# deryrahman/image-caption-emotion-indonesia

Hardware: AMD Instinct MI355X
Metric: images/sec (train step) + NLL loss match, batch=64 ResNet152+FactoredLSTM-512 (higher is better)
Workload: dtype f32 (trunk: operands as 2 f16 pieces each, 3 MFMA products per multiply, f32 accumulate; decoder: large products as 3 bf16 pieces per operand, 6 MFMA products per multiply, the rest f32 MFMA; the persistent LSTM kernel the trunk's split-f16 scheme)

## Files before the change

image-caption-emotion-indonesia_amd/_lib.py:

```python
import ctypes as C
import os

_HERE = os.path.dirname(os.path.abspath(__file__))
LIB_PATH = os.path.join(_HERE, "libcapnet_hip.so")

_f = C.POINTER(C.c_float)
_vp = C.c_void_p
_i = C.c_int
_l = C.c_long
_sz = C.c_size_t
_ip = C.POINTER(C.c_int)

SIGNATURES = {
    "capnet_last_error": (C.c_char_p, []),
    "capnet_abi_version": (_i, []),
    "capnet_sgemm": (_i, [_i, _i, _i, _i, _i, _vp, _l, _vp, _l, _vp, _l, _vp, _i, _i, _l, _l, _l,
                          _l, _i, _vp]),
    "capnet_sgemm_b3": (_i, [_i, _i, _i, _i, _i, _vp, _l, _vp, _l, _vp, _l, _vp, _i, _i, _l, _l, _l, _l, _vp, _sz, _vp]),
    "capnet_sgemm_b3_eligible": (_i, [_i, _i, _i, _i, _i, _vp, _l, _vp, _l, _vp, _l, _vp, _i, _l, _l, _l, _l]),
    "capnet_sgemm_splitk": (_i, [_i, _i, _i, _i, _i, _vp, _l, _vp, _l, _vp, _l, _vp, _i, _vp, _sz, _vp]),
    "capnet_sgemm_splitk_fused": (_i, [_i, _i, _i, _i, _i, _vp, _l, _vp, _l, _vp, _l, _vp, _i, _vp, _sz, _vp, _sz, _vp]),
    "capnet_colsum": (_i, [_vp, _l, _i, _i, _vp, _i, _vp]),
    "capnet_argmax_rows": (_i, [_vp, _i, _i, _i, _vp, _vp]),
    "capnet_resize_u8": (_i, [_vp, _i, _i, _vp, _vp, _i, _i, _vp, _vp, _i, _vp, _vp, _i, _vp]),
    "capnet_crop_flip_normalize": (_i, [_vp, _i, _i, _i, _vp, _vp, _i, _i, _f, _f, _vp]),
    "capnet_topk_correct": (_i, [_vp, _l, _i, _i, _vp, _i, _vp, _vp, _vp]),
    "capnet_beam_topk": (_i, [_vp, _l, _i, _i, _vp, _i, _vp, _vp, _vp]),
    "capnet_beam_topk_batched": (_i, [_vp, _l, _i, _vp, _vp, _i, _vp, _vp, _vp]),
    "capnet_beam_state_bytes": (_sz, [_i, _i, _i]),
    "capnet_beam_init": (_i, [_vp, _i, _i, _i, C.c_longlong, _vp, _vp]),
    "capnet_beam_advance": (_i, [_vp, _vp, _l, _i, _i, _i, _i, _i, C.c_longlong, _vp, _vp, _vp]),
    "capnet_beam_finish": (_i, [_vp, _i, _i, _i, C.c_longlong, _vp, _vp, _vp]),
    "capnet_beam_live": (_i, [_vp, _i, _i, _i, C.POINTER(_vp), C.POINTER(_vp), C.POINTER(_vp)]),
    "capnet_att_step_fwd": (_i, [_vp, _vp, _vp, _vp, _l, _vp, _vp, _i, _i, _i, _i, _vp, _vp, _i, _i,
                                 _vp, _vp, _l, _vp, _vp]),
    "capnet_trunk_create": (_i, [_i, _i, _i, C.POINTER(_vp)]),
    "capnet_trunk_destroy": (None, [_vp]),
    "capnet_trunk_workspace_bytes": (_sz, [_vp]),
    "capnet_trunk_num_convs": (_i, [_vp]),
    "capnet_trunk_final_side": (_i, [_vp]),
    "capnet_trunk_flops": (C.c_double, [_vp]),
    "capnet_trunk_conv_flops": (C.c_double, [_vp, _i]),
    "capnet_trunk_conv_shape": (_i, [_vp, _i, _ip, _ip, _ip, _ip, _ip]),
    "capnet_trunk_forward": (_i, [_vp, _vp, C.POINTER(_vp), C.POINTER(_vp), C.POINTER(_vp),
                                  C.POINTER(_vp), C.POINTER(_vp), _i, C.c_float, C.c_float, _vp,
                                  _vp, _vp, _ip, _vp, _vp]),
    "capnet_trunk_set_tail_balance": (_i, [_vp, _i]),
    "capnet_trunk_update_running": (_i, [_vp, _vp, C.POINTER(_vp), C.POINTER(_vp), C.c_float, _vp]),
    "capnet_pack_conv_weight": (_i, [_vp, _vp, _i, _i, _i, _i, _i, _vp]),
    "capnet_adaptive_pool_replicate": (_i, [_vp, _vp, _i, _i, _i, _i, _vp]),
    "capnet_conv2d_fwd": (_i, [_vp, _l, _l, _l, _l, _vp, _i, _vp, _vp, _vp, _i, _vp, _vp, _i, _i,
                               _i, _i, _i, _i, _i, _i, _i, _i, _vp]),
    "capnet_trunk_conv_kmajor": (_i, [_vp, _i]),
    "capnet_trunk_conv_tile_n": (_i, [_vp, _i]),
    "capnet_pack_conv_weight_kmajor": (_i, [_vp, _vp, _i, _i, _i, _i, _i, _vp]),
    "capnet_conv2d_fwd_kmajor": (_i, [_vp, _l, _l, _l, _vp, _i, _vp, _vp, _vp, _i, _vp, _vp, _i, _i,
                                      _i, _i, _i, _i, _i, _i, _i, _i, _vp, _vp]),
    "capnet_sgemm_nt_dma_eligible": (_i, [_i, _i, _i, _vp, _l, _vp, _l, _vp, _l]),
    "capnet_sgemm_nt_dma": (_i, [_i, _i, _i, _vp, _l, _vp, _vp, _vp, _vp]),
    "capnet_conv1x1_tiles_m": (_i, [_l]),
    "capnet_conv1x1_fwd_dma": (_i, [_vp, _l, _l, _l, _vp, _vp, _vp, _vp, _i, _i, _i, _i, _i, _i, _vp, _vp,
                                    _vp, _i, _vp]),
    "capnet_conv1x1_f16x3_weight_words": (_sz, [_i, _i]),
    "capnet_conv1x1_f16x3_bn": (_i, [_l, _i]),
    "capnet_conv1x1_f16x3_pack": (_i, [_vp, _vp, _i, _i, _i, _vp]),
    "capnet_conv1x1_fwd_f16x3": (_i, [_vp, _l, _l, _l, _vp, _i, _vp, _vp, _vp, _i, _vp, _vp, _i, _i, _i, _i, _i,
                                      _i, _vp, _vp, _vp, _i, _vp]),
    "capnet_conv3x3_fwd_patch": (_i, [_vp, _vp, _i, _vp, _vp, _vp, _i, _vp, _vp, _i, _i, _i, _i, _i, _i, _vp]),
    "capnet_conv1x1_fwd_tail": (_i, [_vp, _vp, _vp, _vp, _vp, _vp, _vp, _vp, _i, _vp, _vp, _vp, _l, _i, _i, _vp]),
    "capnet_conv2d_fwd_f16x3_scaled": (_i, [_vp, _l, _l, _l, _vp, _i, _vp, _vp, _vp, _i, _vp, _vp, _i, _i, _i, _i, _i,
                                            _i, _i, _i, _i, _vp]),
    "capnet_conv3x3_fwd_patch_scaled": (_i, [_vp, _vp, _i, _vp, _vp, _vp, _i, _vp, _vp, _i, _i, _i, _i, _i, _i, _i, _vp]),
    "capnet_conv1x1_fwd_tail_scaled": (_i, [_vp, _vp, _vp, _vp, _vp, _vp, _vp, _vp, _i, _vp, _vp, _vp, _l, _i, _i, _i, _vp]),
    "capnet_conv_stem_f16x3_weight_words": (_sz, []),
    "capnet_conv_stem_f16x3_part_rows": (_i, [_i, _i, _i]),
    "capnet_conv_stem_f16x3_pack": (_i, [_vp, _vp, _vp]),
    "capnet_conv_stem_fwd_f16x3": (_i, [_vp, _l, _l, _l, _vp, _vp, _vp, _vp, _i, _i, _i, _vp]),
    "capnet_conv_f16x3_weight_words": (_sz, [_i, _i, _i]),
    "capnet_conv_f16x3_pack": (_i, [_vp, _vp, _i, _i, _i, _i, _vp]),
    "capnet_conv2d_fwd_f16x3": (_i, [_vp, _l, _l, _l, _vp, _i, _vp, _vp, _vp, _i, _vp, _vp, _i, _i, _i, _i, _i,
                                     _i, _i, _i, _vp, _vp, _vp, _i, _vp]),
    "capnet_conv_kmajor_slab_floats": (_sz, [_i, _i, _i, _i]),
    "capnet_conv_kmajor_plan": (None, [_i, _i, _i, _i, _ip]),
    "capnet_conv_kmajor_tiles_m": (_i, [_i, _i, _i, _i]),
    "capnet_conv_tiles_m": (_i, [_i, _i, _i]),
    "capnet_bn_finalize": (_i, [_vp, _vp, _i, _i, _l, _vp, _vp, _vp, _vp, C.c_float, C.c_float,
                                _vp, _vp, _vp]),
    "capnet_bn_add_relu": (_i, [_vp, _vp, _vp, _vp, _vp, _vp, _vp, _l, _i, _vp]),
    "capnet_bn_relu_maxpool": (_i, [_vp, _vp, _vp, _vp, _i, _i, _i, _i, _vp]),
    "capnet_global_avgpool": (_i, [_vp, _vp, _i, _i, _i, _vp]),
    "capnet_bn1d_fwd": (_i, [_vp, _i, _i, _vp, _vp, _vp, _vp, _i, C.c_float, C.c_float, _vp, _vp,
                             _vp, _vp]),
    "capnet_bn1d_bwd": (_i, [_vp, _vp, _i, _i, _vp, _vp, _vp, _vp, _vp, _vp, _vp]),
    "capnet_seq_saved_floats": (_sz, [_ip]),
    "capnet_seq_saved_ints": (_sz, [_ip]),
    "capnet_seq_saved_cell_offset": (_sz, [_ip]),
    "capnet_seq_fwd_scratch_floats": (_sz, [_ip]),
    "capnet_seq_bwd_scratch_floats": (_sz, [_ip]),
    "capnet_seq_forward": (_i, [_ip, _ip, C.POINTER(C.c_ubyte), _vp, _vp, _vp, C.POINTER(_vp),
                                _vp, _vp, C.c_float, C.c_ulonglong, _i, _vp, _vp, _vp, _vp, _vp,
                                _vp]),
    "capnet_seq_backward": (_i, [_ip, _ip, _vp, _vp, _vp, _vp, _vp, C.POINTER(_vp), C.c_float,
                                 C.c_ulonglong, _i, _vp]),
    "capnet_seq_forward_stacked": (_i, [_ip, _i, _ip, _vp, _vp, _vp, _vp, C.POINTER(_vp), _vp, _vp, C.c_float, C.c_ulonglong, _i,
                                        C.POINTER(_vp), C.POINTER(_vp), _vp, C.POINTER(_vp), _vp, _vp]),
    "capnet_seq_backward_stacked": (_i, [_ip, _i, _ip, _vp, C.POINTER(_vp), C.POINTER(_vp), C.POINTER(_vp), _vp, C.POINTER(_vp),
                                         C.POINTER(_vp), C.c_float, C.c_ulonglong, _i, _vp]),
    "capnet_att_saved_floats": (_sz, [_ip]),
    "capnet_att_saved_ints": (_sz, [_ip]),
    "capnet_att_fwd_scratch_floats": (_sz, [_ip]),
    "capnet_att_bwd_scratch_floats": (_sz, [_ip]),
    "capnet_att_seq_forward": (_i, [_ip, _ip, C.POINTER(C.c_ubyte), _vp, _vp, _vp, C.POINTER(_vp),
                                    _vp, _vp, C.c_float, C.c_ulonglong, _i, _vp, _vp, _vp, _vp, _vp,
                                    _vp, _vp]),
    "capnet_att_seq_backward": (_i, [_ip, _ip, _vp, _vp, _vp, _vp, C.POINTER(_vp), _vp, _vp, _vp,
                                     C.POINTER(_vp), C.c_float, C.c_ulonglong, _i, _vp]),
    "capnet_att_stacked_saved_floats": (_sz, [_ip, _i]),
    "capnet_att_stacked_saved_ints": (_sz, [_ip, _i]),
    "capnet_att_stacked_fwd_scratch_floats": (_sz, [_ip, _i]),
    "capnet_att_stacked_bwd_scratch_floats": (_sz, [_ip, _i]),
    "capnet_att_seq_forward_stacked": (_i, [_ip, _i, _ip, C.POINTER(C.c_ubyte), _vp, _vp, _vp, C.POINTER(_vp), _vp, _vp,
                                            C.c_float, C.c_ulonglong, _i, C.POINTER(_vp), C.POINTER(_vp), _vp,
                                            C.POINTER(_vp), _vp, _vp, _vp]),
    "capnet_att_seq_backward_stacked": (_i, [_ip, _i, _ip, _vp, _vp, C.POINTER(_vp), _vp, C.POINTER(_vp), C.POINTER(_vp),
                                             C.POINTER(_vp), _vp, C.POINTER(_vp), C.POINTER(_vp), C.c_float,
                                             C.c_ulonglong, _i, _vp]),
    "capnet_embedding_fwd": (_i, [_vp, _i, _vp, _i, _i, _vp, _vp, _vp]),
    "capnet_lstm_pointwise_fwd": (_i, [_vp, _vp, _vp, _vp, _i, _i, _i, _vp]),
    "capnet_stacked_decode_step": (_i, [_i, _i, _i, _i, _i, _vp, _vp, C.POINTER(_vp), C.POINTER(_vp), _vp, _vp, _vp, _vp,
                                        _vp]),
    "capnet_stacked_decode_step_cell": (_i, [_i, _i, _i, _i, _i, _i, _vp, _vp, C.POINTER(_vp), C.POINTER(_vp), _vp, _vp,
                                             _vp, _vp, _vp]),
    "capnet_stacked_decode_step_gather": (_i, [_i, _i, _i, _i, _i, _i, _vp, _vp, C.POINTER(_vp), C.POINTER(_vp), _vp, _vp,
                                               _vp, _vp, _vp, _vp]),
    "capnet_stacked_decode_step_groups": (_i, [_i, _i, _i, _i, _i, _i, _i, _vp, _vp, C.POINTER(_vp), C.POINTER(_vp), _vp, _vp,
                                               _vp, _vp, _vp, _vp]),
    "capnet_stacked_decode_step_tables": (_i, [_i, _i, _i, _i, _i, _i, _i, _vp, C.POINTER(_vp), C.POINTER(_vp), C.POINTER(_vp),
                                               _vp, _vp, _vp, _vp, _vp, _vp]),
    "capnet_vocab_argmax_ws_bytes": (_sz, [_i, _i]),
    "capnet_vocab_argmax_groups_ws_bytes": (_sz, [_i, _i, _i]),
    "capnet_vocab_argmax_groups": (_i, [_vp, C.POINTER(_vp), C.POINTER(_vp), _i, _i, _i, _i, _vp, _vp, _vp]),
    "capnet_vocab_argmax": (_i, [_vp, _vp, _vp, _i, _i, _i, _vp, _vp, _vp]),
    "capnet_lstm_greedy_decode_ws_bytes": (_sz, [_i, _i, _i, _i]),
    "capnet_lstm_greedy_decode": (_i, [_i, _i, _i, _i, _i, _i, _vp, _vp, _vp, C.POINTER(_vp), C.POINTER(_vp), _vp, _vp, _vp,
                                       _vp, _vp, _vp, _vp, _vp]),
    "capnet_lstm_greedy_decode_groups_ws_bytes": (_sz, [_i, _i, _i, _i, _i]),
    "capnet_lstm_greedy_decode_groups": (_i, [_i, _i, _i, _i, _i, _i, _i, _vp, C.POINTER(_vp), C.POINTER(_vp), C.POINTER(_vp),
                                              C.POINTER(_vp), C.POINTER(_vp), _vp, _vp, _vp, _vp, _vp, _vp]),
    "capnet_beam_decode_ws_bytes": (_sz, [_i, _i, _i, _i, _i, _i]),
    "capnet_beam_decode": (_i, [_i, _i, _i, _i, _i, _i, _i, _i, C.c_longlong, C.c_longlong, _vp, C.POINTER(_vp),
                                C.POINTER(_vp), _vp, _vp, _vp, _vp, _vp, _sz, _i, _vp, _vp, C.POINTER(_i), _vp, _vp]),
    "capnet_beam_decode_groups": (_i, [_i, _i, _i, _i, _i, _i, _i, _i, _i, C.c_longlong, C.c_longlong, _vp, C.POINTER(_vp),
                                       C.POINTER(_vp), _vp, _vp, _vp, _vp, _vp, _sz, _i, _vp, _vp, C.POINTER(_i), _vp, _vp]),
    "capnet_vocab_topk_ws_bytes": (_sz, [_i, _i, _i]),
    "capnet_vocab_topk": (_i, [_vp, _vp, _vp, _i, _i, _i, _i, _vp, _vp, _vp, _vp, _vp]),
    "capnet_sample_uniform": (C.c_float, [C.c_ulonglong, C.c_uint, C.c_uint, C.c_uint]),
    "capnet_vocab_sample_ws_bytes": (_sz, [_i, _i]),
    "capnet_vocab_sample": (_i, [_vp, _vp, _vp, _i, _i, _i, C.c_float, C.c_ulonglong, C.c_uint, C.c_uint, _vp, _vp, _vp, _vp]),
    "capnet_vocab_sample_greedy": (_i, [_vp, _vp, _vp, _i, _i, _i, C.c_float, C.c_ulonglong, C.c_uint, C.c_uint, _vp, _vp, _vp, C.c_uint, _vp]),
    "capnet_sample_pick": (_i, [_vp, _vp, _i, _i, _i, C.c_float, C.c_ulonglong, C.c_uint, C.c_uint, _vp, _vp, _vp]),
    "capnet_sample_pick_greedy": (_i, [_vp, _vp, _i, _i, _i, C.c_float, C.c_ulonglong, C.c_uint, C.c_uint, _vp, _vp, C.c_uint, _vp]),
    "capnet_sample_rows": (_i, [_vp, _i, _l, _i, C.c_float, C.c_ulonglong, C.c_uint, C.c_uint, _vp, _vp, _vp]),
    "capnet_sample_rows_greedy": (_i, [_vp, _i, _l, _i, C.c_float, C.c_ulonglong, C.c_uint, C.c_uint, _vp, _vp, C.c_uint, _vp]),
    "capnet_sample_decode_ws_bytes": (_sz, [_i, _i, _i, _i, _i]),
    "capnet_sample_decode": (_i, [_i, _i, _i, _i, _i, _i, _i, _vp, _vp, _vp, C.POINTER(_vp), C.POINTER(_vp), _vp, _vp, _vp,
                                  C.c_float, _i, C.c_ulonglong, _vp, _vp, _vp, _vp, _vp, _vp]),
    "capnet_sample_decode_greedy": (_i, [_i, _i, _i, _i, _i, _i, _i, _vp, _vp, _vp, C.POINTER(_vp), C.POINTER(_vp), _vp, _vp, _vp,
                                  C.c_float, _i, C.c_ulonglong, _vp, _vp, _vp, _vp, _vp, C.c_uint, _vp]),
    "capnet_att_sample_decode_ws_bytes": (_sz, [_i] * 10),
    "capnet_att_sample_decode": (_i, [_i] * 11 + [_vp] * 8 + [C.POINTER(_vp), C.POINTER(_vp), _vp, _vp, _vp, C.c_float, _i,
                                                            C.c_ulonglong, _vp, _vp, _sz, _vp, _vp, _vp, _vp, _vp]),
    "capnet_att_sample_decode_greedy": (_i, [_i] * 11 + [_vp] * 8 + [C.POINTER(_vp), C.POINTER(_vp), _vp, _vp, _vp, C.c_float, _i,
                                                            C.c_ulonglong, _vp, _vp, _sz, _vp, _vp, _vp, _vp, C.c_uint, _vp]),
    "capnet_nucleus_rows": (_i, [_vp, _i, _l, _i, C.c_float, C.c_float, C.c_ulonglong, C.c_uint, C.c_uint, _vp, _vp, _vp]),
    "capnet_nucleus_rows_greedy": (_i, [_vp, _i, _l, _i, C.c_float, C.c_float, C.c_ulonglong, C.c_uint, C.c_uint, _vp, _vp, C.c_uint, _vp]),
    "capnet_nucleus_pick": (_i, [_vp, _vp, _i, _i, _i, C.c_float, C.c_float, C.c_ulonglong, C.c_uint, C.c_uint, _vp, _vp, _vp]),
    "capnet_nucleus_pick_greedy": (_i, [_vp, _vp, _i, _i, _i, C.c_float, C.c_float, C.c_ulonglong, C.c_uint, C.c_uint, _vp, _vp, C.c_uint, _vp]),
    "capnet_sample_decode_nucleus_ws_bytes": (_sz, [_i, _i, _i, _i, _i]),
    "capnet_sample_decode_nucleus": (_i, [_i, _i, _i, _i, _i, _i, _i, _vp, _vp, _vp, C.POINTER(_vp), C.POINTER(_vp), _vp, _vp, _vp,
                                          C.c_float, _i, C.c_float, C.c_ulonglong, _vp, _vp, _sz, _vp, _vp, _vp, _vp, _vp]),
    "capnet_sample_decode_nucleus_greedy": (_i, [_i, _i, _i, _i, _i, _i, _i, _vp, _vp, _vp, C.POINTER(_vp), C.POINTER(_vp), _vp, _vp, _vp,
                                          C.c_float, _i, C.c_float, C.c_ulonglong, _vp, _vp, _sz, _vp, _vp, _vp, _vp, C.c_uint, _vp]),
    "capnet_att_sample_decode_nucleus_ws_bytes": (_sz, [_i] * 10),
    "capnet_att_sample_decode_nucleus": (_i, [_i] * 11 + [_vp] * 8 + [C.POINTER(_vp), C.POINTER(_vp), _vp, _vp, _vp, C.c_float, _i,
                                                                    C.c_float, C.c_ulonglong, _vp, _vp, _sz, _vp, _vp, _vp, _vp,
                                                                    _vp]),
    "capnet_att_sample_decode_nucleus_greedy": (_i, [_i] * 11 + [_vp] * 8 + [C.POINTER(_vp), C.POINTER(_vp), _vp, _vp, _vp, C.c_float, _i,
                                                                    C.c_float, C.c_ulonglong, _vp, _vp, _sz, _vp, _vp, _vp, _vp,
                                                                    C.c_uint, _vp]),
    "capnet_vocab_topk_groups_ws_bytes": (_sz, [_i, _i, _i, _i]),
    "capnet_vocab_topk_groups": (_i, [_vp, C.POINTER(_vp), C.POINTER(_vp), _i, _i, _i, _i, _i, _vp, _vp, _vp, _vp, _vp]),
    "capnet_beam_advance_topk": (_i, [_vp, _vp, _vp, _vp, _i, _i, _i, _i, _i, C.c_longlong, _vp, _vp, _vp]),
    "capnet_lstm_beam_decode_ws_bytes": (_sz, [_i, _i, _i, _i, _i, _i, _i]),
    "capnet_lstm_beam_decode": (_i, [_i, _i, _i, _i, _i, _i, _i, _i, C.c_longlong, C.c_longlong, _vp, _vp, C.POINTER(_vp),
                                     C.POINTER(_vp), _vp, _vp, _vp, _vp, _vp, _sz, _i, _i, _vp, _vp, C.POINTER(_i), _vp, _vp]),
    "capnet_lstm_beam_decode_groups_ws_bytes": (_sz, [_i, _i, _i, _i, _i, _i, _i, _i]),
    "capnet_lstm_beam_decode_groups": (_i, [_i, _i, _i, _i, _i, _i, _i, _i, _i, C.c_longlong, C.c_longlong, C.POINTER(_vp),
                                            C.POINTER(_vp), C.POINTER(_vp), C.POINTER(_vp), C.POINTER(_vp), _vp, _vp, _vp, _sz,
                                            _i, _i, _vp, _vp, C.POINTER(_i), _vp, _vp]),
    "capnet_att_decode_supported": (_i, [_i, _i, _i, _i, _i, _i, _i]),
    "capnet_att_decode_step_ws_bytes": (_sz, [_i, _i, _i, _i, _i, _i]),
    "capnet_att_decode_step": (_i, [_i] * 10 + [_vp] * 8 + [C.POINTER(_vp), C.POINTER(_vp), _vp, _vp, _vp, _vp, _vp, _vp, _sz,
                                                          _vp, _vp]),
    "capnet_att_decode_step_groups": (_i, [_i] * 11 + [_vp] * 8 + [C.POINTER(_vp), C.POINTER(_vp), _vp, _vp, _vp, _vp, _vp, _vp,
                                                                 _sz, _vp, _vp]),
    "capnet_att_beam_decode_ws_bytes": (_sz, [_i] * 10),
    "capnet_att_beam_decode": (_i, [_i] * 11 + [C.c_longlong, C.c_longlong] + [_vp] * 7 + [C.POINTER(_vp), C.POINTER(_vp), _vp,
                                                                                           _vp, _vp, _vp, _vp, _sz, _i, _vp, _vp,
                                                                                           C.POINTER(_i), _vp, _vp]),
    "capnet_att_beam_decode_groups": (_i, [_i] * 12 + [C.c_longlong, C.c_longlong] + [_vp] * 7 + [C.POINTER(_vp), C.POINTER(_vp),
                                                                                                  _vp, _vp, _vp, _vp, _vp, _sz,
                                                                                                  _i, _vp, _vp, C.POINTER(_i),
                                                                                                  _vp, _vp]),
    "capnet_beam_trace_bytes": (_sz, [_i, _i, _i]),
    "capnet_beam_advance_traced": (_i, [_vp, _vp, _vp, _l, _i, _i, _i, _i, _i, C.c_longlong, _vp, _vp, _vp]),
    "capnet_beam_finish_traced": (_i, [_vp, _vp, _i, _i, _i, C.c_longlong, _vp, _vp, _vp, _vp]),
    "capnet_att_decode_step_alphas": (_i, [_i] * 11 + [_vp] * 8 + [C.POINTER(_vp), C.POINTER(_vp), _vp, _vp, _vp, _vp, _vp, _vp,
                                                                 _sz, _vp, _vp, _vp]),
    "capnet_att_beam_decode_alphas_ws_bytes": (_sz, [_i] * 11),
    "capnet_att_beam_decode_alphas": (_i, [_i] * 12 + [C.c_longlong, C.c_longlong] + [_vp] * 7 + [C.POINTER(_vp), C.POINTER(_vp),
                                                                                                  _vp, _vp, _vp, _vp, _vp, _sz,
                                                                                                  _i, _vp, _vp, C.POINTER(_i),
                                                                                                  _vp, _vp, _vp]),
    "capnet_beam_nbest": (_i, [_vp, _i, _i, _i, C.c_float, _vp, _vp, _vp, _vp, _vp]),
    "capnet_beam_nbest_traced": (_i, [_vp, _vp, _i, _i, _i, C.c_float, _vp, _vp, _vp, _vp, _vp, _vp]),
    "capnet_beam_decode_ws_beam_offset": (_sz, [_i] * 8),
    "capnet_att_beam_decode_alphas_ws_trace_offset": (_sz, [_i] * 11),
    "capnet_att_beam_decode_alphas_ws_hist_offset": (_sz, [_i] * 11),
    "capnet_alpha_gather": (_i, [_vp, _vp, _i, _i, _i, _i, _vp, _vp]),
    "capnet_lstm_wfrag_floats": (_sz, [_i]),
    "capnet_lstm_pack_wfrag": (_i, [_vp, _vp, _i, _i, _vp]),
    "capnet_lstm_step_fused": (_i, [_vp, _vp, _vp, _l, _vp, _vp, _vp, _i, _i, _i, _vp]),
    "capnet_lstm_step_fused_stamped": (_i, [_vp, _vp, _vp, _l, _vp, _vp, _vp, _i, _i, _vp, _vp]),
    "capnet_lstm_step_fused_supported": (_i, [_i, _i]),
    "capnet_lstm_persist_supported": (_i, [_i, _i]),
    "capnet_lstm_persist_w_floats": (_sz, []),
    "capnet_lstm_persist_ctl_ints": (_sz, []),
    "capnet_lstm_persist_pack": (_i, [_vp, _vp, _i, _vp]),
    "capnet_lstm_persist_run": (_i, [_vp, _vp, _vp, _vp, _ip, _i, _i, _i, _i, _i, _vp, _vp, _vp, _vp]),
    "capnet_xent_fwd": (_i, [_vp, _l, _i, _i, _vp, _vp, _vp, _vp, _vp, _vp]),
    "capnet_xent_bwd": (_i, [_vp, _l, _i, _i, _vp, _vp, _vp, _vp, _l, _vp]),
    "capnet_att_loss_fwd": (_i, [_vp, _vp, _i, _i, _i, C.c_float, _vp, _vp, _vp]),
    "capnet_att_loss_bwd": (_i, [_vp, _vp, _i, _i, _i, C.c_float, _vp, _vp]),
    "capnet_policy_xent_fwd": (_i, [_vp, _l, _i, _i, _vp, _vp, _i, _ip, _i, _vp, _vp, _vp, _vp, _vp, _vp]),
    "capnet_policy_xent_bwd": (_i, [_vp, _l, _i, _i, _vp, _vp, _vp, _i, _ip, _i, _vp, _vp, _l, _vp]),
    "capnet_bleu_rows": (_i, [_vp, _l, _i, _i, C.c_longlong, C.c_longlong, _i, _vp, _vp, _i, _i, _i, C.POINTER(C.c_double), _i,
                              _vp, _vp, _vp]),
    "capnet_cider_rows": (_i, [_vp, _l, _i, _i, C.c_longlong, C.c_longlong, _i, _vp, _vp, _vp, _i, _i, _i, C.POINTER(_vp),
                               C.POINTER(_vp), _ip, C.c_double, C.c_double, _vp, _vp, _vp, _vp]),
    "capnet_clamp_adam": (_i, [_i, C.POINTER(_vp), C.POINTER(_vp), C.POINTER(_vp),
                               C.POINTER(_vp), C.POINTER(_l), _ip, C.c_float, C.c_float,
                               C.c_float, C.c_float, C.c_float, _i, _vp, _vp]),
    "capnet_lstm_persist_set_mode": (_i, [_i]),
    "capnet_att_set_chain_mode": (_i, [_i]),
    "capnet_lstm_pointwise_bwd": (_i, [_vp, _vp, _vp, _vp, _vp, _vp, _i, _i, _i, _vp]),
    "capnet_conv1x1_fwd_areg": (_i, [_vp, _vp, _i, _vp, _vp, _vp, _i, _vp, _vp, _l, _i, _i, _i, _vp]),
    "capnet_trunk_set_timing": (_i, [_vp, _i]),
    "capnet_trunk_time_next_pass": (_i, [_vp]),
    "capnet_trunk_collect_timing": (_i, [_vp, C.POINTER(C.c_double), C.POINTER(_l),
                                         C.POINTER(C.c_double)]),
    "capnet_packed_targets": (_i, [_vp, _i, _i, _ip, _vp, _vp]),
    "capnet_fused_block_weight_words": (_sz, [_i, _i, _i]),
    "capnet_fused_block_pack": (_i, [_vp, _vp, _i, _i, _i, _vp]),
    "capnet_fused_block_stats_floats": (_sz, [_l, _i]),
    "capnet_fused_block_stats": (_i, [_vp, _vp, _vp, _vp, _l, _i, _i, _vp, _vp, _vp, _vp, C.c_float, C.c_float, _vp, _vp, _vp,
                                      _vp, _vp]),
    "capnet_fused_block_tiles": (_i, [_l, _i]),
    "capnet_fused_block_forward": (_i, [_vp] * 14 + [_l, _i, _i, _i, _vp, _vp]),
    "capnet_comm_unique_id": (_i, [_vp]),
    "capnet_comm_create": (_i, [_vp, _i, _i, C.POINTER(_vp)]),
    "capnet_comm_destroy": (_i, [_vp]),
    "capnet_allreduce_grads": (_i, [_vp, _vp, _l, _vp]),
    "capnet_err_word_exchange": (_i, [_vp, _vp, _i, _vp]),
    "capnet_count_skipped": (_i, [_vp, _vp, _vp]),
    "capnet_pack_tensors": (_i, [_i, C.POINTER(_vp), C.POINTER(_l), _vp, _i, C.c_float, _vp]),
    "capnet_clamp": (_i, [_vp, _l, C.c_float, C.c_float, _vp]),
}


class CapnetError(RuntimeError):
    pass


_lib = None


def lib():
    global _lib
    if _lib is None:
        if not os.path.exists(LIB_PATH):
            raise CapnetError(
                "libcapnet_hip.so is not built (%s). Run `python -c 'import __graft_entry__ as g; "
                "g.build()'` or `make -C image-caption-emotion-indonesia_amd/csrc`. There is no "
                "CPU fallback." % LIB_PATH)
        l = C.CDLL(LIB_PATH)
        for name, (res, args) in SIGNATURES.items():
            fn = getattr(l, name)
            fn.restype = res
            fn.argtypes = args
        _lib = l
    return _lib


def check(status, what=""):
    if status != 0:
        msg = lib().capnet_last_error()
        raise CapnetError("%s failed (status %d): %s" %
                          (what or "capnet call", status, msg.decode() if msg else "?"))


def ptr(t):
    if t is None:
        return None
    return C.c_void_p(t.data_ptr())


def ptr_array(tensors):
    arr = (C.c_void_p * len(tensors))()
    for k, t in enumerate(tensors):
        arr[k] = None if t is None else t.data_ptr()
    return arr


def int_array(vals):
    return (C.c_int * len(vals))(*[int(v) for v in vals])


def current_stream():
    import torch
    return C.c_void_p(torch.cuda.current_stream().cuda_stream)
```

image-caption-emotion-indonesia_amd/csrc/capi.cpp:

```cpp
#include "../../include/capnet.h"

#include "common.h"
#include "kernels.h"

using namespace capnet;

static inline hipStream_t S(capnet_stream_t s) { return reinterpret_cast<hipStream_t>(s); }

static SeqDims to_dims(const int* d) {
  SeqDims r;
  r.B = d[0]; r.T = d[1]; r.steps = d[2]; r.N = d[3]; r.E = d[4]; r.F = d[5]; r.H = d[6];
  r.V = d[7]; r.has_features = d[8]; r.cell = d[9];
  return r;
}

static bool weight_used(int cell, int i) { return cell == kCellFactored || i == 0 || i == 4 || i == 24 || i == 28; }
template <class Weights>
static void to_weights(const float* const* weights, Weights& w) {
  for (int g = 0; g < 4; ++g) {
    w.Vw[g] = weights[0 + g];  w.Vb[g] = weights[4 + g];
    w.Sw[g] = weights[8 + g];  w.Sb[g] = weights[12 + g];
    w.Uw[g] = weights[16 + g]; w.Ub[g] = weights[20 + g];
    w.Ww[g] = weights[24 + g]; w.Wb[g] = weights[28 + g];
  }
// ... 1087 lines not shown
int capnet_att_sample_decode_nucleus_greedy(int cell, int nlayers, int n, int m, int P, int A, int C, int E, int H, int V,
                                            int steps, const long long* start_tokens, const float* att1, const float* feat,
                                            const float* emb, const float* wz, const float* bz, const float* w_full,
                                            const float* b_full, const float* const* wcat, const float* const* beff,
                                            const float* Cw, const float* Cb, const float* state0, float temperature,
                                            int top_k, float top_p, unsigned long long seed, void* workspace, float* slab,
                                            size_t slab_floats, long long* ids, float* logp, float* state_out, int* err_flag,
                                            unsigned greedy_stride, capnet_stream_t stream) {
  return att_sample_decode_nucleus_tail(cell, nlayers, n, m, P, A, C, E, H, V, steps, start_tokens, att1, feat, emb, wz, bz,
                                        w_full, b_full, wcat, beff, Cw, Cb, state0, temperature, top_k, top_p, seed,
                                        workspace, slab, slab_floats, ids, logp, state_out, err_flag, stream, greedy_stride);
}

size_t capnet_att_beam_decode_alphas_ws_bytes(int nlayers, int groups, int n, int k, int P, int A, int C, int E, int H, int V,
                                              int max_steps) {
  return att_beam_decode_alphas_ws_bytes(nlayers, groups, n, k, P, A, C, E, H, V, max_steps);
}

int capnet_att_beam_decode_alphas(int cell, int nlayers, int groups, int n, int k, int P, int A, int C, int E, int H, int V,
                                  int max_steps, long long start_token, long long end_token, const float* att1,
                                  const float* feat, const float* emb, const float* wz, const float* bz, const float* w_full,
                                  const float* b_full, const float* const* wcat, const float* const* beff, const float* Cw,
                                  const float* Cb, const float* state0, void* workspace, float* slab, size_t slab_floats,
                                  int poll_every, long long* seqs, int* lengths, int* steps_run, int* err_flag,
                                  capnet_stream_t stream, float* alphas) {
  return att_beam_decode_entry(cell, nlayers, groups, n, k, P, A, C, E, H, V, max_steps, start_token, end_token, att1, feat, emb, wz,
                               bz, w_full, b_full, wcat, beff, Cw, Cb, state0, workspace, slab, slab_floats, poll_every, seqs,
                               lengths, steps_run, err_flag, stream, true, alphas);
}

int capnet_lstm_pointwise_bwd(const float* gates, const float* c, const float* c_prev, const float* dh, float* dc_io,
                              float* dpre, int b, int H, int cell, capnet_stream_t stream) {
  CAPNET_REQUIRE(gates && c && dh && dc_io && dpre && b >= 0 && H > 0, "lstm_pointwise_bwd: bad argument");
  CAPNET_REQUIRE(cell == kCellFactored || cell == kCellLSTM, "lstm_pointwise_bwd: unknown cell %d", cell);
  const bool f = cell == kCellFactored;
  return lstm_pointwise_bwd(gates, 4L * H, c, c_prev, dh, nullptr, dc_io, dpre, 4L * H, b, b, H, 0, 1, f ? 2 : 3, f ? 3 : 2,
                            f ? 0 : 1, S(stream), 0, 0);
}
size_t capnet_lstm_wfrag_floats(int H) { return lstm_wfrag_floats(H); }
int capnet_lstm_pack_wfrag(const float* w_cat, float* w_frag, int H, int cell, capnet_stream_t stream) {
  CAPNET_REQUIRE(cell == kCellFactored || cell == kCellLSTM, "lstm_pack_wfrag: unknown cell %d", cell);
  return cell == kCellFactored ? lstm_pack_wfrag(w_cat, w_frag, H, 0, 1, 2, 3, S(stream))
                               : lstm_pack_wfrag(w_cat, w_frag, H, 0, 1, 3, 2, S(stream));
}
int capnet_lstm_step_fused(const float* h_prev, const float* w_cat, float* gates, long ldg,
                           const float* c_prev, float* c_out, float* h_out, int b, int H, int cell,
                           capnet_stream_t stream) {
  CAPNET_REQUIRE(cell == kCellFactored || cell == kCellLSTM, "lstm_step_fused: unknown cell %d", cell);
  if (cell == kCellFactored)
    return lstm_step_fused(h_prev, w_cat, gates, ldg, c_prev, c_out, h_out, b, H, 0, 1, 2, 3, 0, S(stream));
  return lstm_step_fused(h_prev, w_cat, gates, ldg, c_prev, c_out, h_out, b, H, 0, 1, 3, 2, 1, S(stream));
}
int capnet_lstm_step_fused_stamped(const float* h_prev, const float* w_frag, float* gates, long ldg,
                                   const float* c_prev, float* c_out, float* h_out, int b, int H,
                                   unsigned long long* stamps, capnet_stream_t stream) {
  return lstm_step_fused(h_prev, w_frag, gates, ldg, c_prev, c_out, h_out, b, H, 0, 1, 2, 3, 0,
                         S(stream), stamps);
}
int capnet_lstm_step_fused_supported(int b, int H) { return lstm_step_fused_supported(b, H) ? 1 : 0; }

int capnet_lstm_persist_supported(int b, int H) { return lstm_persist_supported(b, H) ? 1 : 0; }
int capnet_lstm_persist_set_mode(int mode) { return lstm_persist_set_mode(mode); }
size_t capnet_lstm_persist_w_floats(void) { return lstm_persist_w_floats(); }
size_t capnet_lstm_persist_ctl_ints(void) { return lstm_persist_ctl_ints(); }
int capnet_lstm_persist_pack(const float* w_cat, float* w_img, int cell, capnet_stream_t stream) {
  CAPNET_REQUIRE(cell == kCellFactored || cell == kCellLSTM, "lstm_persist_pack: unknown cell %d", cell);
  return cell == kCellFactored ? lstm_persist_pack(w_cat, w_img, 0, 1, 2, 3, S(stream))
                               : lstm_persist_pack(w_cat, w_img, 0, 1, 3, 2, S(stream));
}
int capnet_lstm_persist_run(const float* w_img, float* gates, float* cell_states, float* hiddens,
                            const int* batch_sizes, int t0, int t1, int H, int cell, int segment,
                            int* ctl, int* err_flag, unsigned long long* stamps,
                            capnet_stream_t stream) {
  CAPNET_REQUIRE(cell == kCellFactored || cell == kCellLSTM, "lstm_persist_run: unknown cell %d", cell);
  CAPNET_REQUIRE(batch_sizes && t1 > 0 && t1 <= kMaxSteps, "lstm_persist_run: bad steps");
  int off[kMaxSteps + 1];
  off[0] = 0;
  for (int t = 0; t < t1; ++t) off[t + 1] = off[t] + batch_sizes[t];
  const bool f = cell == kCellFactored;
  return lstm_persist_run(w_img, gates, cell_states, hiddens, off, batch_sizes, t0, t1, H, 0, 1,
                          f ? 2 : 3, f ? 3 : 2, f ? 0 : 1, segment, ctl, err_flag, S(stream), stamps);
}

size_t capnet_seq_saved_floats(const int* dims) { return seq_saved_floats(to_dims(dims)); }
size_t capnet_seq_saved_ints(const int* dims) { return seq_saved_ints(to_dims(dims)); }
size_t capnet_seq_saved_cell_offset(const int* dims) { return seq_saved_cell_offset(to_dims(dims)); }
size_t capnet_seq_fwd_scratch_floats(const int* dims) { return seq_fwd_scratch_floats(to_dims(dims)); }
size_t capnet_seq_bwd_scratch_floats(const int* dims) { return seq_bwd_scratch_floats(to_dims(dims)); }

int capnet_seq_forward_stacked(const int* dims, int nlayers, const int* batch_sizes, const unsigned char* tf_mask,
                               const long long* captions, const float* features, const float* emb,
                               const float* const* weights, const float* Cw, const float* Cb, float dropout_p,
                               unsigned long long seed, int training, float* const* saved, int* const* saved_i,
                               float* scratch, float* const* hiddens, int* err_flag, capnet_stream_t stream) {
  CAPNET_REQUIRE(dims && weights && nlayers >= 1 && nlayers <= 8, "seq_forward_stacked: null dims / weights or layers %d", nlayers);
  const SeqDims d = to_dims(dims);
  CAPNET_REQUIRE(d.cell == kCellFactored || d.cell == kCellLSTM, "seq_forward_stacked: unknown cell %d", d.cell);
  SeqWeights w[8];
  for (int l = 0; l < nlayers; ++l) {
    for (int i = 0; i < 32; ++i)
      CAPNET_REQUIRE(!weight_used(d.cell, i) || weights[32 * l + i], "seq_forward_stacked: weight %d of layer %d is null", i, l);
    to_weights(weights + 32 * l, w[l]);
  }
  return seq_forward_stacked(d, nlayers, batch_sizes, tf_mask, captions, features, emb, w, Cw, Cb, dropout_p, seed, training,
                             saved, saved_i, scratch, hiddens, err_flag, S(stream));
}

int capnet_seq_backward_stacked(const int* dims, int nlayers, const int* batch_sizes, const float* d_hiddens,
                                const float* const* hiddens, const float* const* saved, const int* const* saved_i,
                                float* scratch, float* const* dh_work, float* const* grads, float dropout_p,
                                unsigned long long seed, int training, capnet_stream_t stream) {
  CAPNET_REQUIRE(dims && grads && nlayers >= 1 && nlayers <= 8, "seq_backward_stacked: null dims / grads or layers %d", nlayers);
  SeqGrads g[8];
  for (int l = 0; l < nlayers; ++l) to_grads(grads + 9 * l, g[l]);
  return seq_backward_stacked(to_dims(dims), nlayers, batch_sizes, d_hiddens, hiddens, saved, saved_i, scratch, dh_work, g,
                              dropout_p, seed, training, S(stream));
}

int capnet_seq_forward(const int* dims, const int* batch_sizes, const unsigned char* tf_mask,
                       const long long* captions, const float* features, const float* emb,
                       const float* const* weights, const float* Cw, const float* Cb,
                       float dropout_p, unsigned long long seed, int training, float* saved,
                       int* saved_i, float* scratch, float* hiddens, int* err_flag,
                       capnet_stream_t stream) {
  return capnet_seq_forward_stacked(dims, 1, batch_sizes, tf_mask, captions, features, emb, weights, Cw, Cb, dropout_p, seed,
                                    training, &saved, &saved_i, scratch, &hiddens, err_flag, stream);
}

int capnet_seq_backward(const int* dims, const int* batch_sizes, const float* d_hiddens,
                        const float* hiddens, const float* saved, const int* saved_i,
                        float* scratch, float* const* grads, float dropout_p,
                        unsigned long long seed, int training, capnet_stream_t stream) {
  return capnet_seq_backward_stacked(dims, 1, batch_sizes, d_hiddens, &hiddens, &saved, &saved_i, scratch, nullptr, grads,
                                     dropout_p, seed, training, stream);
}

int capnet_att_set_chain_mode(int mode) { return att_set_chain_mode(mode); }
size_t capnet_att_saved_floats(const int* dims) { return att_saved_floats(to_adims(dims)); }
size_t capnet_att_saved_ints(const int* dims) { return att_saved_ints(to_adims(dims)); }
size_t capnet_att_fwd_scratch_floats(const int* dims) { return att_fwd_scratch_floats(to_adims(dims)); }
size_t capnet_att_bwd_scratch_floats(const int* dims) { return att_bwd_scratch_floats(to_adims(dims)); }

int capnet_beam_topk_batched(const float* logits, long ld, int V, const float* prev_scores, const int* meta, int n,
                             float* top_scores, long long* top_index, capnet_stream_t stream) {
  return beam_topk_batched(logits, ld, V, prev_scores, meta, n, top_scores, top_index, S(stream));
}
int capnet_beam_topk(const float* logits, long ld, int rows, int V, const float* prev_scores, int k,
                     float* top_scores, long long* top_index, capnet_stream_t stream) {
  return beam_topk(logits, ld, rows, V, prev_scores, k, top_scores, top_index, S(stream));
}
size_t capnet_beam_state_bytes(int n, int k, int max_steps) { return beam_state_bytes(n, k, max_steps); }
int capnet_beam_init(void* beam, int n, int k, int max_steps, long long start_token, long long* prev_words,
                     capnet_stream_t stream) {
  return beam_init(beam, n, k, max_steps, start_token, prev_words, S(stream));
}
int capnet_beam_advance(void* beam, const float* logits, long ld, int V, int n, int k, int max_steps, int step,
                        long long end_token, long long* next_words, long long* parent_rows, capnet_stream_t stream) {
  return beam_advance(beam, logits, ld, V, n, k, max_steps, step, end_token, next_words, parent_rows, S(stream));
}
int capnet_beam_advance_topk(void* beam, const float* values, const int* index, const float* lse, int V, int n, int k,
                             int max_steps, int step, long long end_token, long long* next_words, long long* parent_rows,
                             capnet_stream_t stream) {
  return beam_advance_topk(beam, values, index, lse, V, n, k, max_steps, step, end_token, next_words, parent_rows, S(stream));
}
int capnet_beam_finish(const void* beam, int n, int k, int max_steps, long long end_token, long long* seqs, int* lengths,
                       capnet_stream_t stream) {
  return beam_finish(beam, n, k, max_steps, end_token, seqs, lengths, S(stream));
}
size_t capnet_beam_trace_bytes(int n, int k, int max_steps) { return beam_trace_bytes(n, k, max_steps); }
int capnet_beam_advance_traced(void* beam, void* trace, const float* logits, long ld, int V, int n, int k, int max_steps,
                               int step, long long end_token, long long* next_words, long long* parent_rows,
                               capnet_stream_t stream) {
  CAPNET_REQUIRE(trace != nullptr, "beam_advance_traced: null trace");
  CAPNET_REQUIRE((size_t)beam % 4 == 0 && (size_t)trace % 4 == 0, "beam_advance_traced: the state and the trace must be 4-byte aligned");
  return beam_advance(beam, logits, ld, V, n, k, max_steps, step, end_token, next_words, parent_rows, S(stream), trace);
}
int capnet_beam_finish_traced(const void* beam, const void* trace, int n, int k, int max_steps, long long end_token,
                              long long* seqs, int* lengths, int* rows, capnet_stream_t stream) {
  CAPNET_REQUIRE(trace && rows, "beam_finish_traced: null trace or rows");
  CAPNET_REQUIRE((size_t)beam % 4 == 0 && (size_t)trace % 4 == 0 && (size_t)rows % 4 == 0,
                 "beam_finish_traced: the state, the trace and the rows must be 4-byte aligned");
  return beam_finish(beam, n, k, max_steps, end_token, seqs, lengths, S(stream), trace, rows);
}
int capnet_beam_nbest(const void* beam, int n, int k, int max_steps, float length_penalty, long long* seqs, int* lengths,
                      float* scores, int* counts, capnet_stream_t stream) {
  return beam_nbest(beam, n, k, max_steps, length_penalty, seqs, lengths, scores, counts, S(stream));
}
int capnet_beam_nbest_traced(const void* beam, const void* trace, int n, int k, int max_steps, float length_penalty,
                             long long* seqs, int* lengths, float* scores, int* counts, int* rows, capnet_stream_t stream) {
  CAPNET_REQUIRE(trace && rows, "beam_nbest_traced: null trace or rows");
  CAPNET_REQUIRE((size_t)beam % 4 == 0 && (size_t)trace % 4 == 0 && (size_t)rows % 4 == 0,
                 "beam_nbest_traced: the state, the trace and the rows must be 4-byte aligned");
  return beam_nbest(beam, n, k, max_steps, length_penalty, seqs, lengths, scores, counts, S(stream), trace, rows);
}
size_t capnet_beam_decode_ws_beam_offset(int nlayers, int n, int k, int H, int V, int max_steps, int fused_topk, int groups) {
  return beam_decode_ws_beam_offset(nlayers, n, k, H, V, max_steps, fused_topk, groups);
}
size_t capnet_att_beam_decode_alphas_ws_trace_offset(int nlayers, int groups, int n, int k, int P, int A, int C, int E, int H,
                                                     int V, int max_steps) {
// ... 250 lines not shown
```

image-caption-emotion-indonesia_amd/csrc/decoder_seq.cpp:

```cpp
#include <vector>

#include "common.h"
#include "kernels.h"

#include "seq_layers.h"

namespace capnet {

namespace seqd {

std::vector<int> step_offsets(const int* batch_sizes, int steps) {
  std::vector<int> off(steps + 1, 0);
  for (int t = 0; t < steps; ++t) off[t + 1] = off[t] + batch_sizes[t];
  return off;
}

std::vector<int> with_state_step(int B, const int* batch_sizes, int steps) {
  std::vector<int> bse(steps + 1, B);
  for (int t = 0; t < steps; ++t) bse[t + 1] = batch_sizes[t];
  return bse;
}

int check_batch_sizes(const char* who, const int* batch_sizes, int steps, int B, int N) {
  CAPNET_REQUIRE(batch_sizes != nullptr, "%s: null batch_sizes", who);
  long n = 0;
  int prev = B;
  for (int t = 0; t < steps; ++t) {
    CAPNET_REQUIRE(batch_sizes[t] > 0 && batch_sizes[t] <= prev,
                   "%s: batch_sizes must be positive and non-increasing (step %d: %d after %d)", who, t, batch_sizes[t], prev);
    prev = batch_sizes[t];
    n += batch_sizes[t];
  }
  CAPNET_REQUIRE(n == N, "%s: sum(batch_sizes)=%ld != N=%d", who, n, N);
  return kOk;
}

int build_row_tables(const std::vector<int>& off, const unsigned char* tf_mask, int has_features, bool lead, int* row_sample,
                     int* row_col, int* row_token, int* prev_row, hipStream_t s) {
  SeqMeta m;
  m.steps = (int)off.size() - 1; m.N = off.back(); m.has_features = has_features;
  for (int t = 0; t <= m.steps; ++t) m.off[t] = off[t];
  if (lead) m.tf[0] = 1;
  for (int t = lead; t < m.steps; ++t) m.tf[t] = tf_mask[t - lead] ? 1 : 0;
  return build_rows(m, row_sample, row_col, row_token, prev_row, s);
}

Layout make_layout(const SeqDims& d) {
  Layout L;
  Carve take, itake;
  const size_t N = d.N, E = d.E, F = d.F, H = d.H;
  L.X = take(N * E);
  L.G = take(N * 4 * H);
  L.Cst = take(N * H);
  L.Wcat = take(4 * H * H);
  L.Wfrag = take(H % 16 == 0 ? lstm_wfrag_floats((int)H) : 4);
  L.Wp = take(H == 512 ? lstm_persist_w_floats() : 4);
  L.bUW = take(4 * H);
  if (d.cell == kCellFactored) {
    L.A1 = take(N * 4 * F);
    L.A2 = take(N * 4 * F);
    L.Vcat = take(4 * F * E);
    L.Scat = take(4 * F * F);
    L.Ucat = take(4 * H * F);
    L.bV = take(4 * F);
    L.bS = take(4 * F);
  } else {
    L.A1 = L.A2 = L.Scat = L.Ucat = L.bV = L.bS = 0;
    L.Vcat = take(4 * H * E);
  }
  L.total = take.o;
  L.row_sample = itake(N);
  L.row_col = itake(N);
  L.row_token = itake(N);
  L.prev_row = itake(N);
  L.ctl = itake(lstm_persist_ctl_ints());
  L.itotal = itake.o;
  return L;
}

BwdLayout make_bwd_layout(const SeqDims& d, int lead) {
  BwdLayout S;
  Carve take;
  const size_t N = d.N, F = d.F, H = d.H;
  const bool fac = d.cell == kCellFactored;
  S.dPre = take(N * 4 * H);
  S.Hprev = take(N * H);
  S.dh_rec = take((size_t)d.B * H);
  S.dc = take((size_t)d.B * H);
  S.dX = take(N * d.E);
  S.dA2 = take(fac ? N * 4 * F : 0);
  S.dA1 = take(fac ? N * 4 * F : 0);
  S.skws = take(kSplitKFloats);
  S.A1c = take(fac && lead ? N * 4 * F : 0);
  S.A2c = take(fac && lead ? N * 4 * F : 0);
  S.total = take.o;
  return S;
}

int check_dims(const SeqDims& d, const int* batch_sizes) {
  CAPNET_REQUIRE(d.B > 0 && d.T > 0 && d.steps > 0 && d.N > 0 && d.E > 0 && d.H > 0 && d.V > 0,
                 "decoder: bad dims B=%d T=%d steps=%d N=%d E=%d H=%d V=%d", d.B, d.T, d.steps, d.N, d.E, d.H, d.V);
  CAPNET_REQUIRE(d.cell == kCellLSTM || d.F > 0, "decoder: factored size");
  RC(check_batch_sizes("decoder", batch_sizes, d.steps, d.B, d.N));
  CAPNET_REQUIRE(d.steps <= d.T + (d.has_features ? 1 : 0),
                 "decoder: %d steps need more caption columns than T=%d", d.steps, d.T);
  return kOk;
}

int copy_d2d(float* dst, const float* src, size_t n, hipStream_t s) {
  CAPNET_HIP_CHECK(hipMemcpyAsync(dst, src, n * sizeof(float), hipMemcpyDeviceToDevice, s));
  return kOk;
}

static size_t nctr(const SkWs& k) { return k.ctr ? kSplitKCounters : 0; }

int chain_fwd(const Chain& c, const float* X, int n, float* A1, float* A2, float* out, long ldo, const float* bias, int accumulate,
              const SkWs& k, hipStream_t s) {
  const int XW = c.XW, F = c.F, H = c.H;
  RC(sgemm_splitk(false, true, n, 4 * F, XW, X, XW, c.Vcat, XW, A1, 4 * F, c.bV, 0, k.ws, k.floats, s, k.ctr, nctr(k)));
  RC(sgemm_splitk_batched(false, true, n, F, F, A1, 4 * F, c.Scat, F, A2, 4 * F, c.bS, 0, 4, F, (long)F * F, F, F, k.ws, k.floats,
                          s, k.ctr, nctr(k)));
  return sgemm_splitk_batched(false, true, n, H, F, A2, 4 * F, c.Ucat, F, out, ldo, bias, accumulate, 4, F, (long)H * F, H,
                              bias ? H : 0, k.ws, k.floats, s, k.ctr, nctr(k));
}

int chain_collapse(const Chain& c, float* US, float* Weff, float* c1, float* bias, const SkWs& k, hipStream_t s) {
  const int XW = c.XW, F = c.F, H = c.H;
  RC(sgemm(false, false, H, F, F, c.Ucat, F, c.Scat, F, US, F, nullptr, 0, 4, (long)H * F, (long)F * F, (long)H * F, 0, 0, s));
  RC(sgemm(false, false, H, XW, F, US, F, c.Vcat, XW, Weff, XW, nullptr, 0, 4, (long)H * F, (long)F * XW, (long)H * XW, 0, 0, s));
  RC(sgemm_splitk_batched(false, true, 1, F, F, c.bV, F, c.Scat, F, c1, F, c.bS, 0, 4, F, (long)F * F, F, F, k.ws, k.floats, s,
                          k.ctr, nctr(k)));
  return sgemm_splitk_batched(false, true, 1, H, F, c1, F, c.Ucat, F, bias, H, nullptr, 1, 4, F, (long)H * F, H, 0, k.ws, k.floats,
                              s, k.ctr, nctr(k));
}

int chain_rows(const Chain& c, const float* X, int n, float* A1, float* A2, const SkWs& k, hipStream_t s) {
  const int XW = c.XW, F = c.F;
  RC(sgemm_splitk(false, true, n, 4 * F, XW, X, XW, c.Vcat, XW, A1, 4 * F, c.bV, 0, k.ws, k.floats, s, k.ctr, nctr(k)));
  return sgemm(false, true, n, F, F, A1, 4 * F, c.Scat, F, A2, 4 * F, c.bS, 0, 4, F, (long)F * F, F, F, 0, s);
}

int chain_bwd_rows(const Chain& c, const float* dG, long ldg, int n, float* dA2, float* dA1, hipStream_t s) {
  const int F = c.F, H = c.H;
  RC(sgemm(false, false, n, F, H, dG, ldg, c.Ucat, F, dA2, 4 * F, nullptr, 0, 4, H, (long)H * F, F, 0, 0, s));
  return sgemm(false, false, n, F, F, dA2, 4 * F, c.Scat, F, dA1, 4 * F, nullptr, 0, 4, F, (long)F * F, F, 0, 0, s);
}

int chain_wgrads(const Chain& c, const float* dG, long ldg, const float* X, const float* A1, const float* A2, const float* dA2,
                 const float* dA1, int n, const ChainGrads& g, hipStream_t s) {
  const int XW = c.XW, F = c.F, H = c.H;
  RC(sgemm(true, false, H, F, n, dG, ldg, A2, 4 * F, g.dUcat, F, nullptr, 0, 4, H, F, (long)H * F, 0, 0, s));
  RC(colsum(dA2, 4 * F, n, 4 * F, g.dbS, 0, s));
  RC(sgemm(true, false, F, F, n, dA2, 4 * F, A1, 4 * F, g.dScat, F, nullptr, 0, 4, F, F, (long)F * F, 0, 0, s));
  RC(colsum(dA1, 4 * F, n, 4 * F, g.dbV, 0, s));
  return sgemm(true, false, 4 * F, XW, n, dA1, 4 * F, X, XW, g.dVcat, XW, nullptr, 0, 1, 0, 0, 0, 0, 0, s);
}

int lstm_input_wgrad(const float* dG, long ldg, const float* X, int XW, int H, int n, float* dWih, hipStream_t s) {
  return sgemm(true, false, 4 * H, XW, n, dG, ldg, X, XW, dWih, XW, nullptr, 0, 1, 0, 0, 0, 0, 0, s);
}

int input_chain(const SeqDims& d, const Layout& L, float* sv, int r0, int r1, const SkWs& k, hipStream_t s) {
  const int n = r1 - r0;
  if (n <= 0) return kOk;
  const int E = d.E, F = d.F, H = d.H;
  const SkWs kn{n <= 128 ? k.ws : nullptr, k.floats, k.ctr};
  const float* X = sv + L.X + (size_t)r0 * E;
  float* G = sv + L.G + (size_t)r0 * 4 * H;
  if (d.cell == kCellFactored)
    return chain_fwd(chain_of(d, L, sv), X, n, sv + L.A1 + (size_t)r0 * 4 * F, sv + L.A2 + (size_t)r0 * 4 * F, G, 4 * H, sv + L.bUW,
                     0, kn, s);
  return sgemm_splitk(false, true, n, 4 * H, E, X, E, sv + L.Vcat, E, G, 4 * H, sv + L.bUW, 0, kn.ws, kn.floats, s, kn.ctr, nctr(kn));
}

int init_state(const float* mean, int B, int H, int C, const UpperInit& w, float* h0, float* c0, const SkWs& k, hipStream_t s) {
  RC(sgemm_splitk(false, true, B, H, C, mean, C, w.init_h_w, C, h0, H, w.init_h_b, 0, k.ws, k.floats, s, k.ctr, nctr(k)));
  return sgemm_splitk(false, true, B, H, C, mean, C, w.init_c_w, C, c0, H, w.init_c_b, 0, k.ws, k.floats, s, k.ctr, nctr(k));
// ... 78 lines not shown
  return kOk;
}

static bool between_layers(int training, float dropout_p) {
  return (training & 1) && !(training & kSeqInputDropoutOnly) && dropout_p > 0.f;
}

SeqDims upper_dims(const SeqDims& d0) {
  SeqDims d = d0;
  d.E = d0.H;
  d.has_features = 0;
  return d;
}
}

SeqDims seq_upper_dims(const SeqDims& d0) { return upper_dims(d0); }

int seq_forward_stacked(const SeqDims& d0, int nlayers, const int* batch_sizes, const unsigned char* tf_mask,
                        const long long* captions, const float* features, const float* emb, const SeqWeights* w,
                        const float* Cw, const float* Cb, float dropout_p, unsigned long long seed, int training,
                        float* const* saved, int* const* saved_i, float* scratch, float* const* hiddens, int* err_flag,
                        hipStream_t s) {
  RC(check_dims(d0, batch_sizes));
  CAPNET_REQUIRE(nlayers >= 1 && nlayers <= 8 && w && saved && saved_i && hiddens, "seq_forward_stacked: bad argument");
  CAPNET_REQUIRE(tf_mask && captions && emb && scratch && err_flag, "seq_forward: null argument");
  CAPNET_REQUIRE(!d0.has_features || features, "seq_forward: features missing");
  CAPNET_REQUIRE(dropout_p >= 0.f && dropout_p < 1.f, "seq_forward: dropout p=%f", dropout_p);
  const int E = d0.E, N = d0.N, H = d0.H;
  bool any_free = false;
  for (int t = 1; t < d0.steps; ++t) any_free |= !tf_mask[t];
  CAPNET_REQUIRE(!any_free || (Cw && Cb), "seq_forward: output projection needed for free-running steps");
  CAPNET_REQUIRE(d0.steps <= kMaxSteps, "seq_forward: %d steps > %d", d0.steps, kMaxSteps);
  const std::vector<int> off = step_offsets(batch_sizes, d0.steps);

  std::vector<LayerCtx> lay(nlayers);
  for (int l = 0; l < nlayers; ++l) {
    CAPNET_REQUIRE(saved[l] && saved_i[l] && hiddens[l], "seq_forward: null buffer of layer %d", l);
    lay[l].d = l == 0 ? d0 : upper_dims(d0);
    lay[l].L = make_layout(lay[l].d);
    lay[l].sv = saved[l]; lay[l].svi = saved_i[l]; lay[l].hid = hiddens[l];
    RC(build_row_tables(off, tf_mask, d0.has_features, false, lay[l].svi + lay[l].L.row_sample, lay[l].svi + lay[l].L.row_col,
                        lay[l].svi + lay[l].L.row_token, lay[l].svi + lay[l].L.prev_row, s));
    RC(pack_layer(lay[l], w[l], batch_sizes, s));
  }
  LayerCtx& c0 = lay[0];
  LayerCtx& top = lay[nlayers - 1];

  CAPNET_HIP_CHECK(hipMemsetAsync(c0.sv + c0.L.X, 0, (size_t)N * E * sizeof(float), s));
  RC(gather_inputs(captions, d0.T, features, emb, E, d0.V, c0.svi + c0.L.row_sample, c0.svi + c0.L.row_col,
                   c0.svi + c0.L.row_token, c0.sv + c0.L.X, E, 0, N, dropout_p, seed, training && dropout_p > 0.f, 0,
                   err_flag, s));
  float* skws = scratch + (size_t)d0.B * d0.V + 64;
  int* skctr = reinterpret_cast<int*>(skws + kSplitKWs);
  const SkWs sk{skws, kSplitKWs, skctr};
  CAPNET_HIP_CHECK(hipMemsetAsync(skctr, 0, kSplitKCounters * sizeof(int), s));
  RC(input_chain(c0.d, c0.L, c0.sv, 0, N, sk, s));
  const Feedback fb{captions, features, emb, Cw, Cb, d0.T, E, d0.V, H, dropout_p, seed, c0.svi + c0.L.row_sample,
                    c0.svi + c0.L.row_col, c0.svi + c0.L.row_token, scratch, err_flag};

  for (int t = 0; t < d0.steps;) {
    int t1 = t + 1;
    while (t1 < d0.steps && tf_mask[t1]) ++t1;
    const int b = batch_sizes[t], r0 = off[t], r1 = off[t1];
    if (t > 0 && !tf_mask[t]) {
      RC(feed_back(fb, top.hid + (size_t)off[t - 1] * H, b, r0, c0.sv + c0.L.X, E, sk, s));
      RC(input_chain(c0.d, c0.L, c0.sv, r0, r0 + b, sk, s));
    }
    for (int l = 0; l < nlayers; ++l) {
      LayerCtx& c = lay[l];
      if (l > 0) {
        RC(rows_dropout(lay[l - 1].hid, c.sv + c.L.X, r0, r1, H, dropout_p, seed, l, between_layers(training, dropout_p), s));
        RC(input_chain(c.d, c.L, c.sv, r0, r1, sk, s));
      }
      RC(recur(c, off, batch_sizes, t, t1, skws, skctr, err_flag, s));
    }
    t = t1;
  }
  return kOk;
}

static int seq_backward_layer(const SeqDims& d, const int* batch_sizes, const float* dH, const float* hiddens,
                              const float* saved, const int* saved_i, float* scratch, const SeqGrads& g,
                              float dropout_p, unsigned long long seed, int training, int layer, float* dH_below,
                              hipStream_t s, int lead = 0, float* dh0 = nullptr, float* dc0 = nullptr) {
  RC(check_dims(d, batch_sizes));
  CAPNET_REQUIRE(dH && hiddens && saved && saved_i && scratch, "seq_backward: null argument");
  CAPNET_REQUIRE(g.dWcat && g.dbUW && g.dVcat && (layer > 0 ? dH_below != nullptr : g.dEmb != nullptr), "seq_backward: null gradient buffer");
  CAPNET_REQUIRE(lead == 0 || (layer > 0 && d.steps > 1 && dh0 && dc0), "seq_backward: leading state step");
  const Layout L = make_layout(d);
  const BwdLayout S = make_bwd_layout(d, lead);
  const int E = d.E, F = d.F, H = d.H, N = d.N;
  const bool fac = d.cell == kCellFactored;
  const GateOrder go = gate_order(d.cell);
  const std::vector<int> off = step_offsets(batch_sizes, d.steps);
  const int R0 = off[lead], Nr = N - R0;
  float *dPre = scratch + S.dPre, *Hprev = scratch + S.Hprev, *dh_rec = scratch + S.dh_rec, *dc = scratch + S.dc;
  float *dX = scratch + S.dX, *dA2 = scratch + S.dA2, *dA1 = scratch + S.dA1, *skws = scratch + S.skws;
  const float* sv = saved;
  CAPNET_HIP_CHECK(hipMemsetAsync(dh_rec, 0, (size_t)d.B * H * sizeof(float), s));
  CAPNET_HIP_CHECK(hipMemsetAsync(dc, 0, (size_t)d.B * H * sizeof(float), s));

  int slabs = 0;
  for (int t = d.steps - 1; t >= lead; --t) {
    const int b = batch_sizes[t], r0 = off[t];
    const int b_next = (t + 1 < d.steps) ? batch_sizes[t + 1] : 0;
    RC(lstm_pointwise_bwd(sv + L.G + (size_t)r0 * 4 * H, 4 * H, sv + L.Cst + (size_t)r0 * H,
                          t > 0 ? sv + L.Cst + (size_t)off[t - 1] * H : nullptr,
                          dH + (size_t)(r0 - R0) * H, slabs > 0 ? skws : dh_rec, dc, dPre + (size_t)r0 * 4 * H,
                          4 * H, b, b_next, H, go.gi, go.gf, go.go, go.gg, go.tanh_out, s, slabs,
                          (long)b_next * H));
    slabs = 0;
    if (t > 0) {
      RC(sgemm_splitk_slabs(false, b, H, 4 * H, dPre + (size_t)r0 * 4 * H, 4 * H, sv + L.Wcat, H, skws,
                            kSplitKFloats, &slabs, s));
      if (slabs == 0)
        RC(sgemm_splitk(false, false, b, H, 4 * H, dPre + (size_t)r0 * 4 * H, 4 * H, sv + L.Wcat, H,
                        dh_rec, H, nullptr, 0, skws, kSplitKFloats, s));
    }
  }
  if (lead) {
    if (slabs) RC(reduce_slabs(skws, slabs, batch_sizes[0], H, dh_rec, H, nullptr, 0, s));
    RC(copy_d2d(dh0, dh_rec, (size_t)batch_sizes[0] * H, s));
    RC(copy_d2d(dc0, dc, (size_t)batch_sizes[0] * H, s));
  }
  const float* X = sv + L.X + (size_t)R0 * E;
  const float* A1 = lead ? scratch + S.A1c : sv + L.A1;
  const float* A2 = lead ? scratch + S.A2c : sv + L.A2;
  const Chain ch = chain_of(d, L, sv);
  if (fac && lead) RC(chain_rows(ch, X, Nr, scratch + S.A1c, scratch + S.A2c, SkWs{skws, kSplitKFloats, nullptr}, s));
  dPre += (size_t)R0 * 4 * H;
  RC(gather_rows(hiddens, saved_i + L.prev_row + R0, Hprev, Nr, H, s));
  RC(sgemm_splitk(true, false, 4 * H, H, Nr, dPre, 4 * H, Hprev, H, g.dWcat, H, nullptr, 0, skws, kSplitKFloats, s));
  RC(colsum(dPre, 4 * H, Nr, 4 * H, g.dbUW, 0, s));
  if (fac) {
    CAPNET_REQUIRE(g.dUcat && g.dScat && g.dbS && g.dbV, "seq_backward: null factored gradient buffer");
    RC(chain_bwd_rows(ch, dPre, 4 * H, Nr, dA2, dA1, s));
    RC(chain_wgrads(ch, dPre, 4 * H, X, A1, A2, dA2, dA1, Nr, ChainGrads{g.dVcat, g.dbV, g.dScat, g.dbS, g.dUcat}, s));
  } else {
    RC(lstm_input_wgrad(dPre, 4 * H, X, E, H, Nr, g.dVcat, s));
  }
  const int K = fac ? 4 * F : 4 * H;
  RC(sgemm_splitk(false, false, Nr, E, K, fac ? dA1 : dPre, K, sv + L.Vcat, E, dX, E, nullptr, 0, skws, kSplitKFloats, s));
  if (layer > 0) return rows_dropout(dX, dH_below, 0, Nr, E, dropout_p, seed, layer, between_layers(training, dropout_p), s);
  CAPNET_HIP_CHECK(hipMemsetAsync(g.dEmb, 0, (size_t)d.V * E * sizeof(float), s));
  if (g.dFeat) CAPNET_HIP_CHECK(hipMemsetAsync(g.dFeat, 0, (size_t)d.B * E * sizeof(float), s));
  return scatter_input_grad(dX, E, N, E, saved_i + L.row_sample, saved_i + L.row_col, saved_i + L.row_token, g.dEmb, g.dFeat, d.V,
                            dropout_p, seed, training && dropout_p > 0.f, s, reinterpret_cast<int*>(skws), kSplitKFloats);
}

int seqd::seq_backward_upper(const SeqDims& d, const int* batch_sizes, const float* dH, const float* hiddens,
                             const float* saved, const int* saved_i, float* scratch, const SeqGrads& g, float dropout_p,
                             unsigned long long seed, int training, int layer, float* dH_below, float* dh0, float* dc0,
                             hipStream_t s) {
  return seq_backward_layer(d, batch_sizes, dH, hiddens, saved, saved_i, scratch, g, dropout_p, seed, training, layer,
                            dH_below, s, 1, dh0, dc0);
}

int seq_backward_stacked(const SeqDims& d0, int nlayers, const int* batch_sizes, const float* dH_top,
                         const float* const* hiddens, const float* const* saved, const int* const* saved_i, float* scratch,
                         float* const* dH_work, const SeqGrads* g, float dropout_p, unsigned long long seed, int training,
                         hipStream_t s) {
  CAPNET_REQUIRE(nlayers >= 1 && nlayers <= 8 && hiddens && saved && saved_i && g && (nlayers == 1 || dH_work),
                 "seq_backward_stacked: bad argument");
  const float* dH = dH_top;
  for (int l = nlayers - 1; l >= 0; --l) {
    const SeqDims d = l == 0 ? d0 : upper_dims(d0);
    float* below = l > 0 ? dH_work[l - 1] : nullptr;
    RC(seq_backward_layer(d, batch_sizes, dH, hiddens[l], saved[l], saved_i[l], scratch, g[l], dropout_p, seed, training, l,
                          below, s));
    dH = below;
  }
  return kOk;
}

}
```

image-caption-emotion-indonesia_amd/csrc/kernels.h:

```cpp
#pragma once
#include <hip/hip_runtime.h>

namespace capnet {

int sgemm(bool ta, bool tb, int M, int N, int K, const float* A, long lda, const float* B,
          long ldb, float* C, long ldc, const float* bias, int accumulate, int batch, long sA,
          long sB, long sC, long sBias, int force_tile, hipStream_t stream);

bool sgemm_b3_eligible(bool ta, bool tb, int M, int N, int K, const float* A, long lda, const float* B, long ldb,
                       const float* C, long ldc, const float* bias, int batch, long sA, long sB, long sC, long sBias);
int sgemm_b3(bool ta, bool tb, int M, int N, int K, const float* A, long lda, const float* B, long ldb, float* C, long ldc,
             const float* bias, int accumulate, int batch, long sA, long sB, long sC, long sBias, hipStream_t stream,
             float* ws = nullptr, size_t ws_floats = 0);

constexpr size_t kSplitKCounters = 1024;
int sgemm_splitk(bool ta, bool tb, int M, int N, int K, const float* A, long lda, const float* B,
                 long ldb, float* C, long ldc, const float* bias, int accumulate, float* ws,
                 size_t ws_floats, hipStream_t stream, int* counters = nullptr, size_t n_counters = 0);
int sgemm_splitk_slabs(bool tb, int M, int N, int K, const float* A, long lda, const float* B, long ldb,
                       float* ws, size_t ws_floats, int* n_slabs, hipStream_t stream);
int sgemm_rows16_slabs(bool tb, int M, int N, int K, const float* A, long lda, const float* B, long ldb, float* ws,
                       size_t ws_floats, int* n_slabs, hipStream_t stream);
int sgemm_splitk_batched(bool ta, bool tb, int M, int N, int K, const float* A, long lda,
                         const float* B, long ldb, float* C, long ldc, const float* bias,
// ... 238 lines not shown
               int* index, float* lse, hipStream_t stream);
size_t vocab_topk_groups_ws_bytes(int groups, int rpg, int k, int V);
int vocab_topk_groups(const float* h, const float* const* w, const float* const* b, int groups, int rpg, int H, int V, int k,
                      void* ws, float* values, int* index, float* lse, hipStream_t stream);
bool vocab_sample_supported(int H);
float sample_uniform_host(unsigned long long seed, unsigned step, unsigned row, unsigned v);
size_t vocab_sample_ws_bytes(int rows, int V);
int vocab_sample(const float* h, const float* w, const float* b, int rows, int H, int V, float inv_T, unsigned long long seed,
                 unsigned step, unsigned row0, void* ws, long long* tok, long long* ids, float* logp, long ld,
                 hipStream_t stream, unsigned greedy_stride = 0);
int sample_pick(const float* values, const int* index, int rows, int k, int V, float inv_T, unsigned long long seed,
                unsigned step, unsigned row0, long long* tok, long long* ids, float* logp, long ld, hipStream_t stream,
                unsigned greedy_stride = 0);
int sample_rows(const float* logits, int rows, long ld_logits, int V, float inv_T, unsigned long long seed, unsigned step,
                unsigned row0, long long* tok, long long* ids, float* logp, long ld, hipStream_t stream, unsigned greedy_stride = 0);
size_t sample_decode_ws_bytes(int nlayers, int rows, int H, int V, int top_k);
int sample_decode(int cell, int nlayers, int rows, int E, int H, int V, int steps, const float* first_inputs,
                  const long long* start_tokens, const float* emb, const float* const* wcat, const float* const* beff,
                  const float* Cw, const float* Cb, const float* state0, float inv_T, int top_k, unsigned long long seed, void* ws,
                  long long* ids, float* logp, float* state_out, int* err_flag, hipStream_t s);
size_t att_sample_decode_ws_bytes(int nlayers, int n, int m, int P, int A, int C, int E, int H, int V, int top_k);
int att_sample_decode(int cell, int nlayers, int n, int m, int P, int A, int C, int E, int H, int V, int steps,
                      const long long* start_tokens, const float* att1, const float* feat, const float* emb, const float* wz,
                      const float* bz, const float* wf, const float* bf, const float* const* wcat, const float* const* beff,
                      const float* Cw, const float* Cb, const float* state0, float inv_T, int top_k, unsigned long long seed,
                      void* ws, float* slab, size_t slab_floats, long long* ids, float* logp, float* state_out, int* err_flag,
                      hipStream_t s);
int nucleus_rows(const float* logits, int rows, long ld_logits, int V, float inv_T, float top_p, unsigned long long seed,
                 unsigned step, unsigned row0, long long* tok, long long* ids, float* logp, long ld, hipStream_t stream,
                 unsigned greedy_stride = 0);
int nucleus_pick(const float* values, const int* index, int rows, int k, int V, float inv_T, float top_p, unsigned long long seed,
                 unsigned step, unsigned row0, long long* tok, long long* ids, float* logp, long ld, hipStream_t stream,
                 unsigned greedy_stride = 0);
size_t sample_decode_nucleus_ws_bytes(int nlayers, int rows, int H, int V, int top_k);
int sample_decode_nucleus(int cell, int nlayers, int rows, int E, int H, int V, int steps, const float* first_inputs,
                          const long long* start_tokens, const float* emb, const float* const* wcat, const float* const* beff,
                          const float* Cw, const float* Cb, const float* state0, float inv_T, int top_k, float top_p,
                          unsigned long long seed, void* ws, float* slab, size_t slab_floats, long long* ids, float* logp,
                          float* state_out, int* err_flag, hipStream_t s, unsigned greedy_stride = 0);
size_t att_sample_decode_nucleus_ws_bytes(int nlayers, int n, int m, int P, int A, int C, int E, int H, int V, int top_k);
int att_sample_decode_nucleus(int cell, int nlayers, int n, int m, int P, int A, int C, int E, int H, int V, int steps,
                              const long long* start_tokens, const float* att1, const float* feat, const float* emb,
                              const float* wz, const float* bz, const float* wf, const float* bf, const float* const* wcat,
                              const float* const* beff, const float* Cw, const float* Cb, const float* state0, float inv_T,
                              int top_k, float top_p, unsigned long long seed, void* ws, float* slab, size_t slab_floats,
                              long long* ids, float* logp, float* state_out, int* err_flag, hipStream_t s,
                              unsigned greedy_stride = 0);
size_t lstm_beam_decode_ws_bytes(int nlayers, int n, int k, int H, int V, int max_steps, int fused_topk);
int lstm_beam_decode(int cell, int nlayers, int n, int k, int E, int H, int V, int max_steps, long long start_token,
                     long long end_token, const float* first_inputs, const float* emb, const float* const* wcat,
                     const float* const* beff, const float* Cw, const float* Cb, const float* state0, void* ws, float* slab,
                     size_t slab_floats, int fused_topk, int poll_every, long long* seqs, int* lengths, int* steps_run,
                     int* err_flag, hipStream_t s);
size_t lstm_beam_decode_groups_ws_bytes(int nlayers, int groups, int n, int k, int H, int V, int max_steps, int fused_topk);
int lstm_beam_decode_groups(int cell, int nlayers, int groups, int n, int k, int E, int H, int V, int max_steps,
                            long long start_token, long long end_token, const float* const* emb, const float* const* wcat,
                            const float* const* beff, const float* const* Cw, const float* const* Cb, const float* state0,
                            void* ws, float* slab, size_t slab_floats, int fused_topk, int poll_every, long long* seqs,
                            int* lengths, int* steps_run, int* err_flag, hipStream_t s);
size_t att_beam_decode_ws_bytes(int nlayers, int n, int k, int P, int A, int C, int E, int H, int V, int max_steps);
int att_beam_decode(int cell, int nlayers, int n, int k, int P, int A, int C, int E, int H, int V, int max_steps,
                    long long start_token, long long end_token, const float* att1, const float* feat, const float* emb,
                    const float* wz, const float* bz, const float* wf, const float* bf, const float* const* wcat,
                    const float* const* beff, const float* Cw, const float* Cb, const float* state0, void* ws, float* slab,
                    size_t slab_floats, int poll_every, long long* seqs, int* lengths, int* steps_run, int* err_flag,
                    hipStream_t s, int groups = 1, float* alphas = nullptr);
size_t att_beam_decode_alphas_ws_bytes(int nlayers, int groups, int n, int k, int P, int A, int C, int E, int H, int V,
                                       int max_steps);
size_t beam_decode_ws_beam_offset(int nlayers, int n, int k, int H, int V, int max_steps, int fused_topk, int groups);
size_t att_beam_decode_alphas_ws_trace_offset(int nlayers, int groups, int n, int k, int P, int A, int C, int E, int H, int V,
                                              int max_steps);
size_t att_beam_decode_alphas_ws_hist_offset(int nlayers, int groups, int n, int k, int P, int A, int C, int E, int H, int V,
                                             int max_steps);
int alpha_gather(const float* hist, const int* rows, int captions, int nk, int max_steps, int P, float* alphas, hipStream_t s);

bool lstm_persist_supported(int b, int H);
size_t lstm_persist_w_floats();
size_t lstm_persist_ctl_ints();
int lstm_persist_pack(const float* Wcat, float* Wp, int gi, int gf, int go, int gg, hipStream_t stream);
int lstm_persist_run(const float* Wp, float* G, float* Cst, float* hiddens, const int* off,
                     const int* batch_sizes, int t0, int t1, int H, int gi, int gf, int go, int gg,
                     int tanh_out, int seg, int* ctl, int* err_flag, hipStream_t stream,
                     unsigned long long* stamps);

int att_step_fwd(const float* att1, const float* feat, const float* att2, float* gate_io, long ldz,
                 const float* wf, const float* bf, int rows, int P, int A, int C,
                 float* alpha_out, float* alphas_bt, int steps, int t, float* awe_out,
                 float* xa_out, long ldx, float* escore, hipStream_t stream);
bool att_beam_step_supported(int E, int C, int A, int P, int k);
int att_beam_step_fwd(const float* att1, const float* feat, const float* z, const long long* parent_rows, const float* wf,
                      const float* bf, const long long* tokens, const float* emb, int V, int E, int n, int k, int P, int A,
                      int C, float* escore, float* xa, int* err_flag, hipStream_t stream, int n_img = 0,
                      float* alpha_out = nullptr);
int att_step_bwd(const float* att1, const float* feat, const float* att2, long ldz2,
                 const float* gate, long ldzg, const float* awe, const float* alpha,
                 const float* wf, float* dxa, long ldx, const float* dalphas_bt, int steps,
                 int t, int rows, int P, int A, int C, float* dalpha_part, float* dgate_out,
                 float* datt2, long ldz, float* de_out, float* dwf_rows, float* dbf_rows,
                 hipStream_t stream, const float* dxa_slabs = nullptr, int n_slabs = 0, int emb_cols = 0);
int att_datt1(const float* att1, const float* att2_rows, long ldz2, const float* de_rows,
              const float* wf, const int* off, int steps, int B, int P, int A, float* datt1,
              hipStream_t stream);

int resize_u8(const unsigned char* src, int Hs, int Ws, unsigned char* tmp, unsigned char* dst, int Ho,
              int Wo, const int* bounds_h, const int* coef_h, int kmax_h, const int* bounds_v,
              const int* coef_v, int kmax_v, hipStream_t stream);
int crop_flip_normalize(const unsigned char* src, int B, int Hs, int Ws, const int* params, float* dst,
                        int Hc, int Wc, const float* mean, const float* stdv, hipStream_t stream);

int xent_fwd(const float* logits, long ld, int N, int V, const long long* targets, float* lse,
             float* row_loss, float* loss, int* err_flag, hipStream_t stream);
int topk_correct(const float* logits, long ld, int N, int V, const long long* targets, int k,
                 int* count, int* err_flag, hipStream_t stream);
int xent_bwd(const float* logits, long ld, int N, int V, const long long* targets,
             const float* lse, const float* gout, float* dlogits, long ldd, hipStream_t stream);
int att_loss_fwd(const float* nll, const float* alphas, int B, int steps, int P, float alpha_c,
                 float* colsum, float* out, hipStream_t stream);
int att_loss_bwd(const float* gout, const float* colsum, int B, int steps, int P, float alpha_c,
                 float* dalphas, hipStream_t stream);
int policy_xent_fwd(const float* logits, long ld, int N, int V, const long long* targets, const float* adv, int B,
                    const int* batch_sizes, int steps, float* lse, float* row_logp, float* caption_logp, float* loss,
                    int* err_flag, hipStream_t stream);
int policy_xent_bwd(const float* logits, long ld, int N, int V, const long long* targets, const float* lse,
                    const float* adv, int B, const int* batch_sizes, int steps, const float* gout, float* dlogits,
                    long ldd, hipStream_t stream);
constexpr int kBleuMaxSteps = 128, kBleuMaxRefs = 16, kBleuRefWords = 4096;
int bleu_rows(const long long* ids, long ld, int rows, int steps, long long start_token, long long end_token, int per_image,
              const int* refs, const int* ref_len, int images, int R, int Lr, const double* weights, int smooth, float* reward,
              int* stats, hipStream_t stream);
int cider_rows(const long long* ids, long ld, int rows, int steps, long long start_token, long long end_token, int per_image,
               const int* refs, const int* ref_len, const double* ref_norm, int images, int R, int Lr, const int* const* keys,
               const double* const* idf, const int* counts, double log_n, double sigma, float* reward, double* parts, int* stats,
               hipStream_t stream);
int lstm_persist_set_mode(int mode);
int clamp_adam(int n_tensors, float* const* params, float* const* grads, float* const* exp_avg,
               float* const* exp_avg_sq, const long* numel, const int* step, float lr, float b1,
               float b2, float eps, float clip, int write_grad, const int* skip_flag, hipStream_t stream);
bool fused_block_shape_ok(long M, int MID);
size_t fused_block_weight_words(int C, int MID, int role);
int fused_block_pack(const float* w, unsigned* img, int C, int MID, int role, hipStream_t stream);
size_t fused_block_stats_floats(long M, int K);
int fused_block_stats(const float* y2, const float* s2, const float* t2, const unsigned* w3img, long M, int MID, int in_exp,
                      const float* gamma, const float* beta, float* running_mean, float* running_var, float momentum, float eps,
                      float* scale, float* shift, float* batch_mean, float* batch_var, float* work, int* err, hipStream_t stream);
int fused_block_tiles(long M, int MID);
int fused_block_forward(const float* y2, const float* s2, const float* t2, const unsigned* w3img, const float* s3, const float* t3,
                        const float* res, const float* sd, const float* td, float* out, const unsigned* w1img, float* y1,
                        float* part_sum, float* part_sq, long M, int MID, int e3, int e1, int* err, hipStream_t stream);
struct Comm;
int comm_unique_id(void* id128);
int comm_create(const void* id128, int rank, int world, Comm** out);
int comm_destroy(Comm* c);
int allreduce_grads(Comm* c, float* flat, long count, hipStream_t stream);
int err_word_exchange(int* err_flag, float* slot, int dir, hipStream_t stream);
int count_skipped(const int* err_flag, int* counter, hipStream_t stream);
int pack_tensors(int n_tensors, float* const* tensors, const long* numel, float* flat, int dir,
                 float scale, hipStream_t stream);
int clamp_inplace(float* x, long n, float lo, float hi, hipStream_t stream);
int bn1d_fwd(const float* x, int B, int C, const float* gamma, const float* beta, float* rmean,
             float* rvar, int train, float momentum, float eps, float* y, float* save_mean,
             float* save_invstd, hipStream_t stream);
int bn1d_bwd(const float* dy, const float* x, int B, int C, const float* gamma,
             const float* save_mean, const float* save_invstd, float* dx, float* dgamma,
             float* dbeta, hipStream_t stream);

constexpr int kCellFactored = 0;
constexpr int kCellLSTM = 1;
constexpr int kSeqInputDropoutOnly = 2;
struct SeqDims {
  int B, T, steps, N, E, F, H, V, has_features, cell;
};
struct SeqWeights {
  const float* Vw[4]; const float* Vb[4];
  const float* Sw[4]; const float* Sb[4];
  const float* Uw[4]; const float* Ub[4];
  const float* Ww[4]; const float* Wb[4];
};
struct SeqGrads {
  float* dVcat; float* dbV; float* dScat; float* dbS; float* dUcat; float* dbUW; float* dWcat;
  float* dEmb; float* dFeat;
};
size_t seq_saved_floats(const SeqDims& d);
size_t seq_saved_ints(const SeqDims& d);
size_t seq_fwd_scratch_floats(const SeqDims& d);
size_t seq_bwd_scratch_floats(const SeqDims& d);
size_t seq_saved_cell_offset(const SeqDims& d);
SeqDims seq_upper_dims(const SeqDims& d0);
int seq_forward_stacked(const SeqDims& d0, int nlayers, const int* batch_sizes, const unsigned char* tf_mask,
                        const long long* captions, const float* features, const float* emb, const SeqWeights* w,
                        const float* Cw, const float* Cb, float dropout_p, unsigned long long seed, int training,
                        float* const* saved, int* const* saved_i, float* scratch, float* const* hiddens, int* err_flag,
                        hipStream_t s);
int seq_backward_stacked(const SeqDims& d0, int nlayers, const int* batch_sizes, const float* dH_top,
                         const float* const* hiddens, const float* const* saved, const int* const* saved_i, float* scratch,
                         float* const* dH_work, const SeqGrads* g, float dropout_p, unsigned long long seed, int training,
                         hipStream_t s);

struct AttDims {
  int B, T, steps, N, E, F, H, V, A, P, C;
  int cell;
};
struct AttWeights {
  const float* Vw[4]; const float* Vb[4];
  const float* Sw[4]; const float* Sb[4];
  const float* Uw[4]; const float* Ub[4];
  const float* Ww[4]; const float* Wb[4];
  const float* init_h_w; const float* init_h_b; const float* init_c_w; const float* init_c_b;
  const float* enc_att_w; const float* enc_att_b;
  const float* dec_att_w; const float* dec_att_b;
  const float* full_att_w; const float* full_att_b;
  const float* f_beta_w; const float* f_beta_b;
};
struct AttGrads {
  float* dVcat; float* dbV; float* dScat; float* dbS; float* dUcat; float* dWz; float* dbz;
  float* dWe; float* dbe; float* dwf; float* dbf; float* dWih; float* dbih; float* dWic;
  float* dbic; float* dEmb;
};
int att_set_chain_mode(int mode);
size_t att_saved_floats(const AttDims& d);
size_t att_saved_ints(const AttDims& d);
size_t att_fwd_scratch_floats(const AttDims& d);
size_t att_bwd_scratch_floats(const AttDims& d);
int att_seq_backward(const AttDims& d, const int* bs, const float* dH, const float* dalphas_bt,
                     const float* hiddens, const float* feat, const AttWeights& w,
                     const float* saved, const int* saved_i, float* scratch, const AttGrads& g,
                     float dropout_p, unsigned long long seed, int training, hipStream_t s);

struct UpperInit { const float* init_h_w; const float* init_h_b; const float* init_c_w; const float* init_c_b; };
struct UpperInitGrads { float* dWih; float* dbih; float* dWic; float* dbic; };
size_t att_stacked_saved_floats(const AttDims& d, int layer);
size_t att_stacked_saved_ints(const AttDims& d, int layer);
size_t att_stacked_fwd_scratch_floats(const AttDims& d, int nlayers);
size_t att_stacked_bwd_scratch_floats(const AttDims& d, int nlayers);
int att_seq_forward_stacked(const AttDims& d, int nlayers, const int* bs, const unsigned char* tf, const long long* captions,
                            const float* feat, const float* emb, const AttWeights& w0, const SeqWeights* wu,
                            const UpperInit* iu, const float* Cw, const float* Cb, float dropout_p, unsigned long long seed,
                            int training, float* const* saved, int* const* saved_i, float* scratch, float* const* hiddens,
                            float* alphas_bt, int* err_flag, hipStream_t s);
int att_seq_backward_stacked(const AttDims& d, int nlayers, const int* bs, const float* dH_top, const float* dalphas_bt,
                             const float* const* hiddens, const float* feat, const AttWeights& w0,
                             const float* const* saved, const int* const* saved_i, float* scratch, float* const* dH_work,
                             const AttGrads& g0, const SeqGrads* gu, const UpperInitGrads* giu, float dropout_p,
                             unsigned long long seed, int training, hipStream_t s);

}
```

image-caption-emotion-indonesia_amd/csrc/lstm_persist.hip:

```cpp
#include <cstdlib>

#include "common.h"
#include "kernels.h"
#include "mfma_core.h"
#include "split_f16.h"

namespace capnet {

constexpr int kPH = 512;
constexpr int kPShards = 8;
constexpr int kPSlots = 32;
constexpr int kPUnits = 16;
constexpr int kPGrid = kPShards * kPSlots;
constexpr int kPMaxRows = 16;
constexpr int kCtlFlags = 0;
constexpr int kCtlXcc = kPGrid * 4;
constexpr int kCtlAbort = kCtlXcc + kPGrid;
constexpr int kCtlInts = 2048;
constexpr int kSpinBound = 1 << 21;

struct PersistArgs {
  const float* Wp;
  float* G;
  float* Cst;
  float* hiddens;
  int* ctl;
  int* err_flag;
  unsigned long long* stamps;
  int t0, t1, cfg, seg;
  int off[kMaxSteps + 1];
  short b[kMaxSteps];
};

__device__ __forceinline__ int ld_sc1_i32(const int* p) {
  return __hip_atomic_load(p, __ATOMIC_RELAXED, __HIP_MEMORY_SCOPE_AGENT);
}
__device__ __forceinline__ void st_sc1_i32(int* p, int v) {
  __hip_atomic_store(p, v, __ATOMIC_RELAXED, __HIP_MEMORY_SCOPE_AGENT);
}
__device__ __forceinline__ void st_sc1_f32(float* p, float v) {
  __hip_atomic_store(p, v, __ATOMIC_RELAXED, __HIP_MEMORY_SCOPE_AGENT);
}
template <int OFF> __device__ __forceinline__ void ld16_sc1(f32x4& dst, const float* p) {
  asm volatile("global_load_dwordx4 %0, %1, off offset:%2 sc1" : "=v"(dst) : "v"(p), "n"(OFF) : "memory");
}
__device__ __forceinline__ void wait_vm0() { asm volatile("s_waitcnt vmcnt(0)" ::: "memory"); }

constexpr int kWExp = 10;
__device__ __forceinline__ void p_split8(const f32x4& x0, const f32x4& x1, h8& hi, h8& lo) {
  unsigned hw[4], lw[4];
  split2(x0[0], x0[1], hw[0], lw[0]);
  split2(x0[2], x0[3], hw[1], lw[1]);
  split2(x1[0], x1[1], hw[2], lw[2]);
  split2(x1[2], x1[3], hw[3], lw[3]);
  const u4 h = {hw[0], hw[1], hw[2], hw[3]}, l = {lw[0], lw[1], lw[2], lw[3]};
  hi = __builtin_bit_cast(h8, h);
  lo = __builtin_bit_cast(h8, l);
}

__device__ __forceinline__ void persist_mfma_group(const h8& ahi, const h8& alo, const f32x4 (&wq)[32], int g,
                                                   f32x4 (&acc)[4]) {
#pragma unroll
  for (int nb = 0; nb < 4; ++nb)
    acc[nb] = __builtin_amdgcn_mfma_f32_16x16x32_f16(__builtin_bit_cast(h8, wq[(4 * nb + g) * 2]), alo, acc[nb], 0, 0, 0);
#pragma unroll
  for (int nb = 0; nb < 4; ++nb)
    acc[nb] = __builtin_amdgcn_mfma_f32_16x16x32_f16(__builtin_bit_cast(h8, wq[(4 * nb + g) * 2 + 1]), ahi, acc[nb], 0, 0, 0);
#pragma unroll
  for (int nb = 0; nb < 4; ++nb)
    acc[nb] = __builtin_amdgcn_mfma_f32_16x16x32_f16(__builtin_bit_cast(h8, wq[(4 * nb + g) * 2]), ahi, acc[nb], 0, 0, 0);
}

template <int N> __device__ __forceinline__ void wait_h_loads(bool stores) {
  if (stores) wait_vmcnt<N + 9>();
  else wait_vmcnt<N + 4>();
}
__device__ __forceinline__ void persist_mfma(const f32x4 (&hv)[8], const f32x4 (&wq)[32], f32x4 (&acc)[4], bool stores) {
#pragma unroll
  for (int nb = 0; nb < 4; ++nb) acc[nb] = f32x4{0.f, 0.f, 0.f, 0.f};
  h8 ahi[2], alo[2];
  wait_h_loads<6>(stores);
  CAPNET_LANDED_IN1(hv[0]);
  CAPNET_LANDED_IN1(hv[1]);
  __builtin_amdgcn_sched_barrier(0);
  p_split8(hv[0], hv[1], ahi[0], alo[0]);
  asm volatile("" : "+v"(ahi[0]), "+v"(alo[0]));
#define CAPNET_PSTAGE(G)                                                                      \
  __builtin_amdgcn_sched_barrier(0);                                                            \
  wait_h_loads<4 - 2 * (G)>(stores);                                                           \
  CAPNET_LANDED_IN1(hv[2 * (G) + 2]);                                                           \
  CAPNET_LANDED_IN1(hv[2 * (G) + 3]);                                                           \
  __builtin_amdgcn_sched_barrier(0);                                                            \
  p_split8(hv[2 * (G) + 2], hv[2 * (G) + 3], ahi[((G) + 1) & 1], alo[((G) + 1) & 1]);           \
  persist_mfma_group(ahi[(G) & 1], alo[(G) & 1], wq, G, acc);                                  \
  asm volatile("" : "+v"(ahi[((G) + 1) & 1]), "+v"(alo[((G) + 1) & 1]));
  CAPNET_PSTAGE(0) CAPNET_PSTAGE(1) CAPNET_PSTAGE(2)
#undef CAPNET_PSTAGE
  persist_mfma_group(ahi[1], alo[1], wq, 3, acc);
}

__device__ __forceinline__ float fast_sigm(float x) {
  return __builtin_amdgcn_rcpf(1.f + __builtin_amdgcn_exp2f(-1.4426950408889634f * x));
}
__device__ __forceinline__ float fast_tanh(float x) {
  return 1.f - 2.f * __builtin_amdgcn_rcpf(1.f + __builtin_amdgcn_exp2f(2.8853900817779268f * x));
}

template <bool DIAG>
__global__ __launch_bounds__(256) void lstm_persist_kernel(const PersistArgs a) {
  constexpr int H = kPH;
  __shared__ __attribute__((aligned(16))) float red[2][4][kPMaxRows][68];
  __shared__ int s_local, s_abort;
  const int tid = threadIdx.x, lane = tid & 63, wave = tid >> 6;
  const int shard = blockIdx.x & 7, slot = blockIdx.x >> 3;
  const int lm = lane & 15, kq = lane >> 4;
  int* ctl = a.ctl;
  const int gi = a.cfg & 3, gf = (a.cfg >> 2) & 3, go = (a.cfg >> 4) & 3, gg = (a.cfg >> 6) & 3;
  const int tanh_out = (a.cfg >> 8) & 1;
  const int u0 = slot * kPUnits;

  f32x4 wq[32];
  {
    const f32x4* wp = reinterpret_cast<const f32x4*>(a.Wp) + ((long)(slot * 4 + wave) * 32) * 64 + lane;
#pragma unroll
    for (int q = 0; q < 32; ++q) wq[q] = wp[(long)q * 64];
  }
  if (tid == 0) {
    s_abort = 0;
    unsigned x;
    asm volatile("s_getreg_b32 %0, hwreg(HW_REG_XCC_ID)" : "=s"(x));
    st_sc1_i32(&ctl[kCtlXcc + shard * kPSlots + slot], (a.seg << 4) | (int)(x & 15));
  }
  if (wave == 0) {
    int spins = 0, ok = 0, same = 0;
    while (true) {
      const int v = ld_sc1_i32(&ctl[kCtlXcc + shard * kPSlots + (lane & 31)]);
      const int mine = __shfl(v, slot, 64);
      ok = __all((v >> 4) == a.seg);
      same = __all(v == mine);
      if (ok) break;
      if (++spins > kSpinBound || ((spins & 255) == 0 && ld_sc1_i32(&ctl[kCtlAbort]) != 0)) break;
      __builtin_amdgcn_s_sleep(4);
    }
    if (a.cfg & 1024) ok = 0;
    if (lane == 0) {
      s_local = ok && same && !(a.cfg & 512);
      if (!ok) {
        s_abort = 1;
        st_sc1_i32(&ctl[kCtlAbort], 1);
        atomicOr(a.err_flag, 4);
      }
    }
  }
  __syncthreads();
  if (s_abort) return;
  const bool local = s_local != 0;
  if (tid == 0 && slot == 0) ctl[kCtlAbort + 1 + shard] = local ? 1 : 2;
  if (tid == 0 && blockIdx.x == 0 && reinterpret_cast<const unsigned*>(a.Wp)[4l * kPH * kPH] != 0u) atomicOr(a.err_flag, 32);

  const int em = tid >> 4, eu = tid & 15;
  const int grow = 8 * em + shard;
  float c_reg = 0.f;
  if (a.t0 > 0 && grow < a.b[a.t0 - 1])
    c_reg = a.Cst[(long)(a.off[a.t0 - 1] + grow) * H + u0 + eu];
  const int* my_flags = ctl + kCtlFlags + (shard * kPSlots + 8 * wave) * 4 + (lane & 31);
  int* out_flag = ctl + kCtlFlags + (shard * kPSlots + slot) * 4 + wave;

  unsigned long long rt0 = 0, mt0 = 0;
  if (DIAG) { rt0 = __builtin_amdgcn_s_memrealtime(); mt0 = __builtin_amdgcn_s_memtime(); }
  int v_off0 = a.off[lane], v_off1 = a.off[64 + lane < kMaxSteps ? 64 + lane : kMaxSteps];
  int v_b0 = a.b[lane], v_b1 = a.b[64 + lane < kMaxSteps ? 64 + lane : kMaxSteps - 1];
  wait_vm0();
  asm volatile("" : "+v"(v_off0), "+v"(v_off1), "+v"(v_b0), "+v"(v_b1));
  auto off_of = [&](int t) { return t < 64 ? __builtin_amdgcn_readlane(v_off0, t) : __builtin_amdgcn_readlane(v_off1, t - 64); };
  auto b_of = [&](int t) { return t < 64 ? __builtin_amdgcn_readlane(v_b0, t) : __builtin_amdgcn_readlane(v_b1, t - 64); };
  f32x4 dgate = {0.f, 0.f, 0.f, 0.f};
  float dcell = 0.f;
  long drow = -1;

  auto st32 = [](float* p, float v) { asm volatile("global_store_dword %0, %1, off" :: "v"(p), "v"(v) : "memory"); };
  auto flush_deferred = [&]() {
    if (drow >= 0) {
      float* gp = a.G + drow * (4 * H) + u0 + eu;
      st32(gp + (long)gi * H, dgate[0]);
      st32(gp + (long)gf * H, dgate[1]);
      st32(gp + (long)go * H, dgate[2]);
      st32(gp + (long)gg * H, dgate[3]);
      st32(a.Cst + drow * H + u0 + eu, dcell);
    }
  };

  for (int t = a.t0; t < a.t1; ++t) {
    unsigned long long ts[6] = {0, 0, 0, 0, 0, 0};
    if (DIAG) ts[0] = __builtin_amdgcn_s_memtime();
    const int bt = b_of(t);
    const int rows_t = (bt - shard + 7) >> 3;
    const int ro = off_of(t);
    const bool evalid = em < rows_t;
    const long erow = ro + (evalid ? grow : 0);
    const bool product = t > 0;
    f32x4 hv[8];
    if (product) {
      if (t > a.t0) {
        int spins = 0;
        while (true) {
          const int v = ld_sc1_i32(my_flags);
          if (__all(v - t >= 0)) break;
          if (++spins > kSpinBound || ((spins & 255) == 0 && ld_sc1_i32(&ctl[kCtlAbort]) != 0)) {
            if (lane == 0) {
              st_sc1_i32(&ctl[kCtlAbort], 1);
              atomicOr(a.err_flag, 4);
            }
            break;
          }
        }
      }
      if (DIAG) ts[1] = __builtin_amdgcn_s_memtime();
      const int rp = off_of(t - 1);
      const float* hrow = a.hiddens + (long)(rp + 8 * lm + shard) * H + 128 * wave + 4 * kq;
      if (lm < rows_t) {
        ld16_sc1<0>(hv[0], hrow);
        ld16_sc1<64>(hv[1], hrow);
        ld16_sc1<128>(hv[2], hrow);
        ld16_sc1<192>(hv[3], hrow);
        ld16_sc1<256>(hv[4], hrow);
        ld16_sc1<320>(hv[5], hrow);
        ld16_sc1<384>(hv[6], hrow);
        ld16_sc1<448>(hv[7], hrow);
      } else {
#pragma unroll
        for (int q = 0; q < 8; ++q) asm volatile("" : "=v"(hv[q]));
      }
    }
    f32x4 pre;
    {
      const float* gp = a.G + erow * (4 * H) + u0 + eu;
      asm volatile("global_load_dword %0, %1, off" : "=v"(pre[0]) : "v"(gp + (long)gi * H) : "memory");
      asm volatile("global_load_dword %0, %1, off" : "=v"(pre[1]) : "v"(gp + (long)gf * H) : "memory");
      asm volatile("global_load_dword %0, %1, off" : "=v"(pre[2]) : "v"(gp + (long)go * H) : "memory");
      asm volatile("global_load_dword %0, %1, off" : "=v"(pre[3]) : "v"(gp + (long)gg * H) : "memory");
    }
    const bool had_deferred = drow >= 0;
    flush_deferred();
    drow = -1;
    __builtin_amdgcn_sched_barrier(0);

    if (product) {
      f32x4 acc[4];
      const bool stores_in_flight = __any(had_deferred);
      persist_mfma(hv, wq, acc, stores_in_flight);
      if (DIAG) ts[2] = __builtin_amdgcn_s_memtime();
      if (lm < rows_t) {
#pragma unroll
        for (int nb = 0; nb < 4; ++nb) *reinterpret_cast<f32x4*>(&red[t & 1][wave][lm][4 * (4 * nb + kq)]) = acc[nb];
      }
    }
    wait_vm0();
    __builtin_amdgcn_sched_barrier(0);
    if (product) {
      __syncthreads();
      if (evalid) {
        f32x4 sum = *reinterpret_cast<const f32x4*>(&red[t & 1][0][em][4 * eu]);
#pragma unroll
        for (int w = 1; w < 4; ++w) sum += *reinterpret_cast<const f32x4*>(&red[t & 1][w][em][4 * eu]);
        pre += sum * (1.f / (float)(1 << kWExp));
      }
    }
    if (DIAG) ts[3] = __builtin_amdgcn_s_memtime();
    if (evalid) {
      const float i = fast_sigm(pre[0]), f = fast_sigm(pre[1]), og = fast_sigm(pre[2]), gt = fast_tanh(pre[3]);
      c_reg = f * c_reg + i * gt;
      const float h = tanh_out ? og * fast_tanh(c_reg) : og * c_reg;
      float* hp = a.hiddens + erow * H + u0 + eu;
      if (local) st32(hp, h);
      else asm volatile("global_store_dword %0, %1, off sc1" :: "v"(hp), "v"(h) : "memory");
      dgate = f32x4{i, f, og, gt};
      dcell = c_reg;
      drow = erow;
    }
    if (t + 1 < a.t1) {
      wait_vm0();
      if (DIAG) ts[4] = __builtin_amdgcn_s_memtime();
      if (lane == 0) {
        if (local) asm volatile("global_store_dword %0, %1, off" :: "v"(out_flag), "v"(t + 1) : "memory");
        else asm volatile("global_store_dword %0, %1, off sc1" :: "v"(out_flag), "v"(t + 1) : "memory");
      }
    }
    if (DIAG) {
      ts[5] = __builtin_amdgcn_s_memtime();
      if (tid == 0) {
        unsigned long long* st = a.stamps + ((long)(t - a.t0) * kPGrid + blockIdx.x) * 8;
#pragma unroll
        for (int k = 0; k < 6; ++k) st[k] = ts[k];
      }
      wait_vm0();
    }
  }
  flush_deferred();
  if (DIAG && tid == 0) {
    unsigned long long* st = a.stamps + (long)(a.t1 - a.t0) * kPGrid * 8 + blockIdx.x * 2;
    st[0] = __builtin_amdgcn_s_memtime() - mt0;
    st[1] = __builtin_amdgcn_s_memrealtime() - rt0;
  }
}

__global__ __launch_bounds__(256) void lstm_persist_pack_kernel(const float* __restrict__ Wcat,
                                                                unsigned* __restrict__ Wp, int g0,
                                                                int g1, int g2, int g3) {
  const int grow[4] = {g0, g1, g2, g3};
  const long total = 2L * kPH * kPH;
  for (long i = (long)blockIdx.x * blockDim.x + threadIdx.x; i < total;
       i += (long)gridDim.x * blockDim.x) {
    const int jp = (int)(i & 3), lane = (int)((i >> 2) & 63);
    long r = i >> 8;
    const int g = (int)(r & 3); r >>= 2;
    const int nb = (int)(r & 3); r >>= 2;
    const int w = (int)(r & 3);
    const int slot = (int)(r >> 2);
    const int n = lane & 15, kq = lane >> 4;
    const int k = 128 * w + 32 * g + 16 * (jp >> 1) + 4 * kq + 2 * (jp & 1);
    const float* src = Wcat + ((long)grow[n & 3] * kPH + 16 * slot + 4 * nb + (n >> 2)) * kPH + k;
    unsigned h, l;
    split2(src[0] * (float)(1 << kWExp), src[1] * (float)(1 << kWExp), h, l);
    const long q = ((long)(slot * 4 + w) * 32 + (4 * nb + g) * 2) * 256 + lane * 4 + jp;
    Wp[q] = h;
    Wp[q + 256] = l;
    const float lim = 65504.f / (float)(1 << kWExp);
    if (!(fabsf(src[0]) <= lim && fabsf(src[1]) <= lim)) Wp[4l * kPH * kPH] = 1u;
  }
}

size_t lstm_persist_w_floats() { return 4ul * kPH * kPH + 4; }
size_t lstm_persist_ctl_ints() { return kCtlInts; }

static int& persist_mode() {
  static int mode = [] { const char* off = getenv("CAPNET_NO_PERSISTENT_LSTM"); return (off && off[0] == '1') ? 1 : 0; }();
  return mode;
}
int lstm_persist_set_mode(int mode) {
  const int old = persist_mode();
  if (mode >= 0) persist_mode() = mode & 7;
  return old;
}

static int persist_device_ok() {
  static int cached = -1;
  if (cached >= 0) return cached;
  int dev = 0, cus = 0, per_cu = 0;
  if (hipGetDevice(&dev) != hipSuccess ||
      hipDeviceGetAttribute(&cus, hipDeviceAttributeMultiprocessorCount, dev) != hipSuccess) {
    (void)hipGetLastError();
    return cached = 0;
  }
  if (hipOccupancyMaxActiveBlocksPerMultiprocessor(&per_cu, (const void*)lstm_persist_kernel<false>, 256,
                                                   0) != hipSuccess) {
    (void)hipGetLastError();
    return cached = 0;
  }
  cached = (cus >= kPGrid && per_cu >= 1) ? 1 : 0;
  return cached;
}

bool lstm_persist_supported(int b, int H) {
  return H == kPH && b >= 1 && b <= 8 * kPMaxRows && !(persist_mode() & 1) && persist_device_ok();
}

int lstm_persist_pack(const float* Wcat, float* Wp, int gi, int gf, int go, int gg, hipStream_t stream) {
  CAPNET_REQUIRE(Wcat && Wp && aligned16(Wp), "lstm_persist_pack: bad argument");
  CAPNET_HIP_CHECK(hipMemsetAsync(Wp + 4l * kPH * kPH, 0, 4 * sizeof(float), stream));
  hipLaunchKernelGGL(lstm_persist_pack_kernel, dim3(1024), dim3(256), 0, stream, Wcat, reinterpret_cast<unsigned*>(Wp), gi, gf,
                     go, gg);
  CAPNET_LAUNCH_CHECK();
  return kOk;
}

int lstm_persist_run(const float* Wp, float* G, float* Cst, float* hiddens, const int* off,
                     const int* batch_sizes, int t0, int t1, int H, int gi, int gf, int go, int gg,
                     int tanh_out, int seg, int* ctl, int* err_flag, hipStream_t stream,
                     unsigned long long* stamps) {
  CAPNET_REQUIRE(Wp && G && Cst && hiddens && off && batch_sizes && ctl && err_flag,
                 "lstm_persist_run: null argument");
  CAPNET_REQUIRE(0 <= t0 && t0 < t1 && t1 <= kMaxSteps, "lstm_persist_run: steps [%d, %d)", t0, t1);
  CAPNET_REQUIRE(seg > 0 && seg < (1 << 26), "lstm_persist_run: segment tag %d", seg);
  const int b0 = batch_sizes[t0 > 0 ? t0 - 1 : t0];
  CAPNET_REQUIRE(lstm_persist_supported(b0, H), "lstm_persist_run: unsupported b=%d H=%d", b0, H);
  CAPNET_REQUIRE(aligned16(Wp) && aligned16(hiddens), "lstm_persist_run: alignment");
  PersistArgs a;
  a.Wp = Wp; a.G = G; a.Cst = Cst; a.hiddens = hiddens; a.ctl = ctl; a.err_flag = err_flag;
  a.stamps = stamps;
  a.t0 = t0; a.t1 = t1; a.seg = seg;
  a.cfg = gi | (gf << 2) | (go << 4) | (gg << 6) | ((tanh_out ? 1 : 0) << 8) | ((persist_mode() & 2) ? 512 : 0) |
          ((persist_mode() & 4) ? 1024 : 0);
  for (int t = 0; t <= t1; ++t) a.off[t] = off[t];
  int prev = 1 << 30;
  for (int t = (t0 > 0 ? t0 - 1 : 0); t < t1; ++t) {
    CAPNET_REQUIRE(batch_sizes[t] >= 1 && batch_sizes[t] <= prev, "lstm_persist_run: batch sizes must not grow");
    prev = batch_sizes[t];
  }
  for (int t = 0; t < t1; ++t) a.b[t] = (short)batch_sizes[t];
  if (stamps) hipLaunchKernelGGL((lstm_persist_kernel<true>), dim3(kPGrid), dim3(256), 0, stream, a);
  else hipLaunchKernelGGL((lstm_persist_kernel<false>), dim3(kPGrid), dim3(256), 0, stream, a);
  CAPNET_LAUNCH_CHECK();
  return kOk;
}

}
```

image-caption-emotion-indonesia_amd/csrc/seq_layers.h:

```cpp
#pragma once
#include <vector>

#include "common.h"
#include "kernels.h"

#define RC(x) do { int _rc = (x); if (_rc) return _rc; } while (0)

namespace capnet {

constexpr size_t kSplitKFloats = 32ull * 64 * 2048;
constexpr size_t kSplitKWs = kSplitKFloats - kSplitKCounters;

namespace seqd {

struct Carve {
  size_t o = 0;
  size_t operator()(size_t n) { const size_t r = o; o += (n + 3) / 4 * 4; return r; }
};

struct GateOrder { int gi, gf, go, gg, tanh_out; };
inline GateOrder gate_order(int cell) { return cell == kCellFactored ? GateOrder{0, 1, 2, 3, 0} : GateOrder{0, 1, 3, 2, 1}; }

std::vector<int> step_offsets(const int* batch_sizes, int steps);
std::vector<int> with_state_step(int B, const int* batch_sizes, int steps);
int check_batch_sizes(const char* who, const int* batch_sizes, int steps, int B, int N);
int build_row_tables(const std::vector<int>& off, const unsigned char* tf_mask, int has_features, bool lead, int* row_sample,
                     int* row_col, int* row_token, int* prev_row, hipStream_t s);

struct SkWs { float* ws; size_t floats; int* ctr; };

struct Chain { const float *Vcat, *Scat, *Ucat, *bV, *bS; int XW, F, H; };
struct ChainGrads { float *dVcat, *dbV, *dScat, *dbS, *dUcat; };
int chain_fwd(const Chain& c, const float* X, int n, float* A1, float* A2, float* out, long ldo, const float* bias, int accumulate,
              const SkWs& k, hipStream_t s);
int chain_collapse(const Chain& c, float* US, float* Weff, float* c1, float* bias, const SkWs& k, hipStream_t s);
int chain_rows(const Chain& c, const float* X, int n, float* A1, float* A2, const SkWs& k, hipStream_t s);
int chain_bwd_rows(const Chain& c, const float* dG, long ldg, int n, float* dA2, float* dA1, hipStream_t s);
int chain_wgrads(const Chain& c, const float* dG, long ldg, const float* X, const float* A1, const float* A2, const float* dA2,
                 const float* dA1, int n, const ChainGrads& g, hipStream_t s);
int lstm_input_wgrad(const float* dG, long ldg, const float* X, int XW, int H, int n, float* dWih, hipStream_t s);

struct Layout {
  size_t X, A1, A2, G, Cst, Vcat, Scat, Ucat, Wcat, Wfrag, Wp, bV, bS, bUW, total;
  size_t row_sample, row_col, row_token, prev_row, ctl, itotal;
};
Layout make_layout(const SeqDims& d);
inline Chain chain_of(const SeqDims& d, const Layout& L, const float* sv) {
  return {sv + L.Vcat, sv + L.Scat, sv + L.Ucat, sv + L.bV, sv + L.bS, d.E, d.F, d.H};
}

int input_chain(const SeqDims& d, const Layout& L, float* sv, int r0, int r1, const SkWs& k, hipStream_t s);

struct LayerCtx {
  SeqDims d;
  Layout L;
  float* sv; int* svi; float* hid;
  bool fused_step = false, persist = false;
  int segment = 0;
};
template <class W>
void add_cell_copies(CopyTable& ct, const W& w, int cell, size_t XW, size_t F, size_t H, float* Vcat, float* Scat, float* Ucat,
                     float* Wrec, float* bV, float* bS, float* brec) {
  if (cell != kCellFactored) {
    ct.add(Vcat, w.Vw[0], 4 * H * XW);
    ct.add(Wrec, w.Ww[0], 4 * H * H);
    ct.add(brec, w.Vb[0], 4 * H, w.Wb[0]);
    return;
  }
  for (int g = 0; g < 4; ++g) {
    ct.add(Vcat + g * F * XW, w.Vw[g], F * XW);
    ct.add(Scat + g * F * F, w.Sw[g], F * F);
    ct.add(Ucat + g * H * F, w.Uw[g], H * F);
    ct.add(Wrec + g * H * H, w.Ww[g], H * H);
    ct.add(bV + g * F, w.Vb[g], F);
    ct.add(bS + g * F, w.Sb[g], F);
    ct.add(brec + g * H, w.Ub[g], H, w.Wb[g]);
  }
}
int pack_layer(LayerCtx& c, const SeqWeights& w, const int* batch_sizes, hipStream_t s);
int recur(LayerCtx& c, const std::vector<int>& off, const int* batch_sizes, int t, int t1, float* skws, int* skctr,
          int* err_flag, hipStream_t s);

int init_state(const float* mean, int B, int H, int C, const UpperInit& w, float* h0, float* c0, const SkWs& k, hipStream_t s);
int init_state_grad(const float* dh0, const float* dc0, const float* mean, int B, int H, int C, const UpperInitGrads& g,
                    hipStream_t s);

struct Feedback {
  const long long* captions;
  const float *features, *emb, *Cw, *Cb;
  int T, E, V, H;
  float dropout_p; unsigned long long seed;
  const int *row_sample, *row_col; int* row_token;
  float* logits; int* err_flag;
};
int feed_back(const Feedback& f, const float* h_prev, int b, int r0, float* X, long ldx, const SkWs& k, hipStream_t s);

struct BwdLayout { size_t dPre, Hprev, dh_rec, dc, dX, dA2, dA1, skws, A1c, A2c, total; };
BwdLayout make_bwd_layout(const SeqDims& d, int lead);

int seq_backward_upper(const SeqDims& d, const int* batch_sizes, const float* dH, const float* hiddens, const float* saved,
                       const int* saved_i, float* scratch, const SeqGrads& g, float dropout_p, unsigned long long seed,
                       int training, int layer, float* dH_below, float* dh0, float* dc0, hipStream_t s);

}
}
```

image-caption-emotion-indonesia_amd/ops.py:

```python
import ctypes as C

import struct
import sys
import weakref

import torch
from torch.autograd.function import once_differentiable

from . import _lib
from ._lib import CapnetError, check, current_stream, int_array, ptr, ptr_array

CELL_FACTORED = 0
CELL_LSTM = 1

_err_flags = {}


def _need_cuda(*tensors):
    for t in tensors:
        if t is None:
            continue
        if not t.is_cuda:
            raise CapnetError("capnet operators run on the GPU only (got a %s tensor); there is "
                              "no CPU fallback" % t.device)
# ... 1719 lines not shown
        out += slots
    return out


def _tf_bytes(tf):
    return (C.c_ubyte * len(tf))(*[1 if x else 0 for x in tf])


def _seq_training(cfg):
    return int(bool(cfg["training"])) | (2 if cfg.get("input_dropout_only") else 0)


class SeqFn(torch.autograd.Function):

    @staticmethod
    def forward(ctx, cfg, captions, features, emb, Cw, Cb, *weights):
        _need_cuda(captions, features, emb, Cw, Cb, *weights)
        captions = _c(captions)
        cell, nl = _seq_args(cfg, captions)
        ws = [_c(w) for w in weights]
        if len(ws) != (32 if cell == CELL_FACTORED else 4) * nl:
            raise CapnetError("the factored cell takes 32 weight tensors per layer, the LSTM cell 4")
        if cell != CELL_FACTORED:
            ws = _lstm_slots(ws)
        emb, Cw, Cb = _c(emb), _c(Cw), _c(Cb)
        dev = emb.device
        bs, tf = cfg["batch_sizes"], cfg["tf_mask"]
        B, T = captions.shape
        V, E = emb.shape
        H, F, N = cfg["hidden_size"], cfg.get("factored_size", 0), sum(bs)
        if features is not None:
            features = _c(features)
            if tuple(features.shape) != (B, E):
                raise CapnetError("features must be [batch, embed_size]")
        dims = [[B, T, len(bs), N, E if l == 0 else H, F, H, V, int(features is not None) if l == 0 else 0, cell]
                for l in range(nl)]
        L = _lib.lib()
        cd = [int_array(d) for d in dims]
        saved = [torch.empty(L.capnet_seq_saved_floats(c), dtype=torch.float32, device=dev) for c in cd]
        saved_i = [torch.empty(L.capnet_seq_saved_ints(c), dtype=torch.int32, device=dev) for c in cd]
        scratch = torch.empty(L.capnet_seq_fwd_scratch_floats(cd[0]), dtype=torch.float32, device=dev)
        hid = [torch.empty((N, H), dtype=torch.float32, device=dev) for _ in range(nl)]
        check(L.capnet_seq_forward_stacked(cd[0], nl, int_array(bs), _tf_bytes(tf), ptr(captions), ptr(features),
                                           ptr(emb), ptr_array(ws), ptr(Cw), ptr(Cb), float(cfg["dropout"]),
                                           int(cfg["seed"]), _seq_training(cfg), ptr_array(saved), ptr_array(saved_i),
                                           ptr(scratch), ptr_array(hid), ptr(err_flag(dev)), current_stream()),
              "capnet_seq_forward_stacked")
        if cfg.get("want_final_state"):
            last = N - bs[-1]
            cst = [saved[l][L.capnet_seq_saved_cell_offset(cd[l]):][:N * H].view(N, H) for l in range(nl)]
            cfg["final_state"] = (torch.stack([h[last:] for h in hid]), torch.stack([c[last:] for c in cst]))
        ctx.cfg, ctx.dims, ctx.has_features = cfg, dims, features is not None
        ctx.save_for_backward(*(saved + saved_i + hid))
        return hid[-1]

    @staticmethod
    @once_differentiable
    def backward(ctx, d_hiddens):
        cfg, dims = ctx.cfg, ctx.dims
        nl = len(dims)
        t = ctx.saved_tensors
        saved, saved_i, hid = t[:nl], t[nl:2 * nl], t[2 * nl:]
        B, T, steps, N, E, F, H, V, _, cell = dims[0]
        dev = saved[0].device
        L = _lib.lib()
        cd = [int_array(d) for d in dims]
        scratch = torch.empty(max(L.capnet_seq_bwd_scratch_floats(c) for c in cd), dtype=torch.float32, device=dev)

        def new(*shape):
            return torch.empty(shape, dtype=torch.float32, device=dev)

        dEmb = new(V, E)
        dFeat = new(B, E) if ctx.has_features else None
        grads, per_layer = [], []
        for l in range(nl):
            El = E if l == 0 else H
            if cell == CELL_FACTORED:
                g = [new(4 * F, El), new(4 * F), new(4, F, F), new(4 * F), new(4, H, F), new(4 * H), new(4 * H, H)]
            else:
                g = [new(4 * H, El), None, None, None, None, new(4 * H), new(4 * H, H)]
            grads += g + [dEmb if l == 0 else None, dFeat if l == 0 else None]
            per_layer.append(g)
        dh_work = [new(N, H) for _ in range(nl - 1)]
        check(L.capnet_seq_backward_stacked(cd[0], nl, int_array(cfg["batch_sizes"]), ptr(_c(d_hiddens)), ptr_array(hid),
                                            ptr_array(saved), ptr_array(saved_i), ptr(scratch),
                                            ptr_array(dh_work) if dh_work else None, ptr_array(grads),
                                            float(cfg["dropout"]), int(cfg["seed"]), _seq_training(cfg), current_stream()),
              "capnet_seq_backward_stacked")
        wg = []
        for g in per_layer:
            wg += _gate_grads(cell, F, H, *g)
        return (None, None, dFeat, dEmb, None, None) + tuple(wg)


class AttSeqFn(torch.autograd.Function):

    @staticmethod
    def forward(ctx, cfg, captions, features, emb, Cw, Cb, *weights):
        _need_cuda(captions, features, emb, Cw, Cb, *weights)
        captions = _c(captions)
        cell, nl = _seq_args(cfg, captions)
        ws = [_c(w) for w in weights]
        if len(ws) != (44 + 36 * (nl - 1) if cell == CELL_FACTORED else 16 + 8 * (nl - 1)):
            raise CapnetError("attention decoder: 44 + 36 (num_layers - 1) weight tensors (factored) / "
                              "16 + 8 (num_layers - 1) (LSTMCell)")
        if cell != CELL_FACTORED:
            upper = []
            for l in range(1, nl):
                u = ws[16 + 8 * (l - 1):16 + 8 * l]
                upper += _lstm_slots(u[:4]) + u[4:]
            ws = _lstm_slots(ws[:4]) + ws[4:16] + upper
        emb, Cw, Cb = _c(emb), _c(Cw), _c(Cb)
        dev = emb.device
        bs, tf = cfg["batch_sizes"], cfg["tf_mask"]
        B, T = captions.shape
        V, E = emb.shape
        H, A = cfg["hidden_size"], cfg["attention_size"]
        F = cfg["factored_size"] if cell == CELL_FACTORED else 4
        features = _c(features)
        if features.dim() != 3 or features.shape[0] != B:
            raise CapnetError("features must be [batch, pixels, feature_size]")
        P, Cf = features.shape[1], features.shape[2]
        N = sum(bs)
        dims = [B, T, len(bs), N, E, F, H, V, A, P, Cf, cell]
        cdims = int_array(dims)
        L = _lib.lib()
        saved = [torch.empty(L.capnet_att_stacked_saved_floats(cdims, l), dtype=torch.float32, device=dev) for l in range(nl)]
        saved_i = [torch.empty(L.capnet_att_stacked_saved_ints(cdims, l), dtype=torch.int32, device=dev) for l in range(nl)]
        scratch = torch.empty(L.capnet_att_stacked_fwd_scratch_floats(cdims, nl), dtype=torch.float32, device=dev)
        hid = [torch.empty((N if l == 0 else B + N, H), dtype=torch.float32, device=dev) for l in range(nl)]
        alphas = torch.empty((B, len(bs), P), dtype=torch.float32, device=dev)
        check(L.capnet_att_seq_forward_stacked(cdims, nl, int_array(bs), _tf_bytes(tf), ptr(captions), ptr(features),
                                               ptr(emb), ptr_array(ws), ptr(Cw), ptr(Cb), float(cfg["dropout"]),
                                               int(cfg["seed"]), int(cfg["training"]), ptr_array(saved), ptr_array(saved_i),
                                               ptr(scratch), ptr_array(hid), ptr(alphas), ptr(err_flag(dev)),
                                               current_stream()), "capnet_att_seq_forward_stacked")
        ctx.cfg, ctx.dims, ctx.nl = cfg, dims, nl
        ctx.save_for_backward(*(saved + saved_i + hid), features, *ws)
        return (hid[0] if nl == 1 else hid[-1][B:]), alphas

    @staticmethod
    @once_differentiable
    def backward(ctx, d_hiddens, d_alphas):
        cfg, dims, nl = ctx.cfg, ctx.dims, ctx.nl
        t = ctx.saved_tensors
        saved, saved_i, hid, features, ws = t[:nl], t[nl:2 * nl], t[2 * nl:3 * nl], t[3 * nl], t[3 * nl + 1:]
        B, T, steps, N, E, F, H, V, A, P, Cf, cell = dims
        dev = features.device
        L = _lib.lib()
        cdims = int_array(dims)
        scratch = torch.empty(L.capnet_att_stacked_bwd_scratch_floats(cdims, nl), dtype=torch.float32, device=dev)

        def new(*shape):
            return torch.empty(shape, dtype=torch.float32, device=dev)

        d_hiddens = _c(d_hiddens) if d_hiddens is not None else torch.zeros((N, H), dtype=torch.float32, device=dev)
        d_alphas = _c(d_alphas) if d_alphas is not None else None
        XW = E + Cf
        if cell == CELL_FACTORED:
            dV, dbV, dS, dbS, dU = new(4 * F, XW), new(4 * F), new(4, F, F), new(4 * F), new(4, H, F)
        else:
            dV, dbV, dS, dbS, dU = new(4 * H, XW), None, None, None, None
        dWz, dbz = new(4 * H + A + Cf, H), new(4 * H + A + Cf)
        dWe, dbe, dwf, dbf = new(A, Cf), new(A), new(1, A), new(1)
        dWih, dbih, dWic, dbic = new(H, Cf), new(H), new(H, Cf), new(H)
        dEmb = new(V, E)
        grads = [dV, dbV, dS, dbS, dU, dWz, dbz, dWe, dbe, dwf, dbf, dWih, dbih, dWic, dbic, dEmb]
        upper = []
        for _ in range(1, nl):
            if cell == CELL_FACTORED:
                g = [new(4 * F, H), new(4 * F), new(4, F, F), new(4 * F), new(4, H, F), new(4 * H), new(4 * H, H)]
# ... 18 lines not shown
```

include/capnet.h:

```cpp
#ifndef CAPNET_H_
#define CAPNET_H_

#include <stddef.h>

#ifdef __cplusplus
extern "C" {
#endif

typedef void* capnet_stream_t;
typedef struct capnet_trunk capnet_trunk_t;

#define CAPNET_OK 0
#define CAPNET_ERR_INVALID_ARG (-1)
#define CAPNET_ERR_HIP (-2)

const char* capnet_last_error(void);
int capnet_abi_version(void);

int capnet_sgemm(int transA, int transB, int M, int N, int K, const float* A, long lda,
                 const float* B, long ldb, float* C, long ldc, const float* bias, int accumulate,
                 int batch, long strideA, long strideB, long strideC, long strideBias,
                 int force_tile, capnet_stream_t stream);
int capnet_sgemm_b3(int transA, int transB, int M, int N, int K, const float* A, long lda, const float* B, long ldb,
                    float* C, long ldc, const float* bias, int accumulate, int batch, long strideA, long strideB,
// ... 104 lines not shown
                            const float* in_scale, const float* in_shift, int relu_in, float* part_sum,
                            float* part_sq, int B, int H, int W, int Cin, int Cout, int k, int stride, int pad,
                            const float* out_scale, const float* out_shift, const float* res, int relu_out,
                            capnet_stream_t stream);

int capnet_conv3x3_fwd_patch(const float* x, const unsigned* image, int bn, float* y, const float* in_scale,
                             const float* in_shift, int relu_in, float* part_sum, float* part_sq, int B, int H, int W,
                             int Cin, int Cout, int shared_chip, capnet_stream_t stream);

int capnet_conv1x1_fwd_tail(const float* y3, const float* s1, const float* t1, const float* res, const float* s2,
                            const float* t2, float* tail_out, const unsigned* image, int bn, float* y, float* part_sum,
                            float* part_sq, long M, int Cin, int Cout, capnet_stream_t stream);
int capnet_conv2d_fwd_f16x3_scaled(const float* x, long sxb, long sxh, long sxw, const unsigned* image, int bn, float* y,
                                   const float* in_scale, const float* in_shift, int relu_in, float* part_sum,
                                   float* part_sq, int B, int H, int W, int Cin, int Cout, int k, int stride, int pad,
                                   int in_exp, capnet_stream_t stream);
int capnet_conv3x3_fwd_patch_scaled(const float* x, const unsigned* image, int bn, float* y, const float* in_scale,
                                    const float* in_shift, int relu_in, float* part_sum, float* part_sq, int B, int H,
                                    int W, int Cin, int Cout, int shared_chip, int in_exp, capnet_stream_t stream);
int capnet_conv1x1_fwd_tail_scaled(const float* y3, const float* s1, const float* t1, const float* res, const float* s2,
                                   const float* t2, float* tail_out, const unsigned* image, int bn, float* y,
                                   float* part_sum, float* part_sq, long M, int Cin, int Cout, int in_exp,
                                   capnet_stream_t stream);

size_t capnet_conv_stem_f16x3_weight_words(void);
int capnet_conv_stem_f16x3_part_rows(int B, int H, int W);
int capnet_conv_stem_f16x3_pack(const float* w_oihw, unsigned* image, capnet_stream_t stream);
int capnet_conv_stem_fwd_f16x3(const float* x, long sxb, long sxc, long sxh, const unsigned* image, float* y,
                               float* part_sum, float* part_sq, int B, int H, int W, capnet_stream_t stream);

int capnet_conv2d_fwd_kmajor(const float* x, long sxb, long sxh, long sxw, const float* w_kmajor,
                             int k_rows, float* y, const float* in_scale, const float* in_shift,
                             int relu_in, float* part_sum, float* part_sq, int B, int H, int W,
                             int Cin, int Cout, int KH, int KW, int stride, int pad, int tile,
                             float* slabs, capnet_stream_t stream);
size_t capnet_conv_kmajor_slab_floats(int M, int Cout, int k_rows, int tile);
void capnet_conv_kmajor_plan(int M, int Cout, int k_rows, int tile, int* out5);
int capnet_conv_kmajor_tiles_m(int M, int Cout, int k_rows, int tile);
int capnet_conv_tiles_m(int M, int Cout, int tile);
int capnet_bn_finalize(const float* part_sum, const float* part_sq, int tiles, int C, long count,
                       const float* gamma, const float* beta, float* running_mean,
                       float* running_var, float momentum, float eps, float* scale, float* shift,
                       capnet_stream_t stream);
int capnet_bn_add_relu(const float* y, const float* s1, const float* t1, const float* res,
                       const float* s2, const float* t2, float* out, long rows, int C,
                       capnet_stream_t stream);
int capnet_bn_relu_maxpool(const float* y, const float* scale, const float* shift, float* out,
                           int B, int H, int W, int C, capnet_stream_t stream);
int capnet_global_avgpool(const float* x, float* out, int B, int HW, int C,
                          capnet_stream_t stream);

int capnet_bn1d_fwd(const float* x, int B, int C, const float* gamma, const float* beta,
                    float* running_mean, float* running_var, int train, float momentum, float eps,
                    float* y, float* save_mean, float* save_invstd, capnet_stream_t stream);
int capnet_bn1d_bwd(const float* dy, const float* x, int B, int C, const float* gamma,
                    const float* save_mean, const float* save_invstd, float* dx, float* dgamma,
                    float* dbeta, capnet_stream_t stream);

size_t capnet_seq_saved_floats(const int* dims);
size_t capnet_seq_saved_ints(const int* dims);
size_t capnet_seq_saved_cell_offset(const int* dims);
size_t capnet_seq_fwd_scratch_floats(const int* dims);
size_t capnet_seq_bwd_scratch_floats(const int* dims);
int capnet_seq_forward(const int* dims, const int* batch_sizes, const unsigned char* tf_mask,
                       const long long* captions, const float* features, const float* emb,
                       const float* const* weights, const float* Cw, const float* Cb,
                       float dropout_p, unsigned long long seed, int training, float* saved,
                       int* saved_i, float* scratch, float* hiddens, int* err_flag,
                       capnet_stream_t stream);
int capnet_seq_backward(const int* dims, const int* batch_sizes, const float* d_hiddens,
                        const float* hiddens, const float* saved, const int* saved_i,
                        float* scratch, float* const* grads, float dropout_p,
                        unsigned long long seed, int training, capnet_stream_t stream);

int capnet_seq_forward_stacked(const int* dims, int nlayers, const int* batch_sizes, const unsigned char* tf_mask,
                               const long long* captions, const float* features, const float* emb,
                               const float* const* weights, const float* Cw, const float* Cb, float dropout_p,
                               unsigned long long seed, int training, float* const* saved, int* const* saved_i,
                               float* scratch, float* const* hiddens, int* err_flag, capnet_stream_t stream);
int capnet_seq_backward_stacked(const int* dims, int nlayers, const int* batch_sizes, const float* d_hiddens,
                                const float* const* hiddens, const float* const* saved, const int* const* saved_i,
                                float* scratch, float* const* dh_work, float* const* grads, float dropout_p,
                                unsigned long long seed, int training, capnet_stream_t stream);

int capnet_att_set_chain_mode(int mode);
size_t capnet_att_saved_floats(const int* dims);
size_t capnet_att_saved_ints(const int* dims);
size_t capnet_att_fwd_scratch_floats(const int* dims);
size_t capnet_att_bwd_scratch_floats(const int* dims);
int capnet_att_step_fwd(const float* att1, const float* feat, const float* att2, float* gate_io,
                        long ldz, const float* w_full, const float* b_full, int rows, int P, int A,
                        int C, float* alpha_out, float* alphas_bt, int steps, int t, float* awe_out,
                        float* xa_out, long ldx, float* scores_ws, capnet_stream_t stream);

int capnet_att_seq_forward(const int* dims, const int* batch_sizes, const unsigned char* tf_mask,
                           const long long* captions, const float* features, const float* emb,
                           const float* const* weights, const float* Cw, const float* Cb,
                           float dropout_p, unsigned long long seed, int training, float* saved,
                           int* saved_i, float* scratch, float* hiddens, float* alphas,
                           int* err_flag, capnet_stream_t stream);
int capnet_att_seq_backward(const int* dims, const int* batch_sizes, const float* d_hiddens,
                            const float* d_alphas, const float* hiddens, const float* features,
                            const float* const* weights, const float* saved, const int* saved_i,
                            float* scratch, float* const* grads, float dropout_p,
                            unsigned long long seed, int training, capnet_stream_t stream);

size_t capnet_att_stacked_saved_floats(const int* dims, int layer);
size_t capnet_att_stacked_saved_ints(const int* dims, int layer);
size_t capnet_att_stacked_fwd_scratch_floats(const int* dims, int nlayers);
size_t capnet_att_stacked_bwd_scratch_floats(const int* dims, int nlayers);
int capnet_att_seq_forward_stacked(const int* dims, int nlayers, const int* batch_sizes, const unsigned char* tf_mask,
                                   const long long* captions, const float* features, const float* emb,
                                   const float* const* weights, const float* Cw, const float* Cb, float dropout_p,
                                   unsigned long long seed, int training, float* const* saved, int* const* saved_i,
                                   float* scratch, float* const* hiddens, float* alphas, int* err_flag,
                                   capnet_stream_t stream);
int capnet_att_seq_backward_stacked(const int* dims, int nlayers, const int* batch_sizes, const float* d_hiddens,
                                    const float* d_alphas, const float* const* hiddens, const float* features,
                                    const float* const* weights, const float* const* saved, const int* const* saved_i,
                                    float* scratch, float* const* dh_work, float* const* grads, float dropout_p,
                                    unsigned long long seed, int training, capnet_stream_t stream);

int capnet_embedding_fwd(const long long* idx, int n, const float* emb, int E, int V, float* out,
                         int* err_flag, capnet_stream_t stream);
int capnet_lstm_pointwise_fwd(float* pre, const float* c_prev, float* c_out, float* h_out, int b,
                              int H, int cell, capnet_stream_t stream);
int capnet_lstm_pointwise_bwd(const float* gates, const float* c, const float* c_prev, const float* dh, float* dc_io,
                              float* dpre, int b, int H, int cell, capnet_stream_t stream);

int capnet_stacked_decode_step(int nlayers, int rows, int E, int H, int V, const long long* tokens, const float* x,
                               const float* const* wcat, const float* const* beff, const float* state_in,
                               float* state_out, float* h_top, int* err_flag, capnet_stream_t stream);

int capnet_stacked_decode_step_cell(int cell, int nlayers, int rows, int E, int H, int V, const long long* tokens,
                                    const float* x, const float* const* wcat, const float* const* beff,
                                    const float* state_in, float* state_out, float* h_top, int* err_flag,
                                    capnet_stream_t stream);

int capnet_stacked_decode_step_gather(int cell, int nlayers, int rows, int E, int H, int V, const long long* tokens,
                                      const float* x, const float* const* wcat, const float* const* beff,
                                      const float* state_in, const long long* parent_rows, float* state_out, float* h_top,
                                      int* err_flag, capnet_stream_t stream);

int capnet_stacked_decode_step_groups(int cell, int nlayers, int groups, int rows_per_group, int E, int H, int V,
                                      const long long* tokens, const float* x, const float* const* wcat,
                                      const float* const* beff, const float* state_in, const long long* parent_rows,
                                      float* state_out, float* h_top, int* err_flag, capnet_stream_t stream);

int capnet_stacked_decode_step_tables(int cell, int nlayers, int groups, int rows_per_group, int E, int H, int V,
                                      const long long* tokens, const float* const* tables, const float* const* wcat,
                                      const float* const* beff, const float* state_in, const long long* parent_rows,
                                      float* state_out, float* h_top, int* err_flag, capnet_stream_t stream);

size_t capnet_vocab_argmax_ws_bytes(int rows, int V);
int capnet_vocab_argmax(const float* h, const float* w, const float* b, int rows, int H, int V, void* workspace,
                        long long* tokens, capnet_stream_t stream);

size_t capnet_vocab_argmax_groups_ws_bytes(int groups, int rows_per_group, int V);
int capnet_vocab_argmax_groups(const float* h, const float* const* w, const float* const* b, int groups, int rows_per_group,
                               int H, int V, void* workspace, long long* tokens, capnet_stream_t stream);

size_t capnet_lstm_greedy_decode_ws_bytes(int nlayers, int rows, int H, int V);
int capnet_lstm_greedy_decode(int nlayers, int rows, int E, int H, int V, int steps, const float* features,
                              const long long* start_tokens, const float* emb, const float* const* wcat,
                              const float* const* beff, const float* Cw, const float* Cb, const float* state0,
                              void* workspace, long long* ids, float* state_out, int* err_flag, capnet_stream_t stream);
// ... 142 lines not shown

int capnet_att_decode_supported(int E, int C, int H, int A, int P, int k, int nlayers);
size_t capnet_att_decode_step_ws_bytes(int n, int k, int P, int A, int C, int E);
int capnet_att_decode_step(int cell, int nlayers, int n, int k, int P, int A, int C, int E, int H, int V, const float* att1,
                           const float* feat, const long long* tokens, const float* emb, const float* wz, const float* bz,
                           const float* w_full, const float* b_full, const float* const* wcat, const float* const* beff,
                           const float* state_in, const long long* parent_rows, float* state_out, float* h_top,
                           void* workspace, float* slab, size_t slab_floats, int* err_flag, capnet_stream_t stream);

int capnet_att_decode_step_groups(int cell, int nlayers, int groups, int n, int k, int P, int A, int C, int E, int H, int V,
                                  const float* att1, const float* feat, const long long* tokens, const float* emb,
                                  const float* wz, const float* bz, const float* w_full, const float* b_full,
                                  const float* const* wcat, const float* const* beff, const float* state_in,
                                  const long long* parent_rows, float* state_out, float* h_top, void* workspace, float* slab,
                                  size_t slab_floats, int* err_flag, capnet_stream_t stream);

size_t capnet_att_beam_decode_ws_bytes(int nlayers, int n, int k, int P, int A, int C, int E, int H, int V, int max_steps);
int capnet_att_beam_decode(int cell, int nlayers, int n, int k, int P, int A, int C, int E, int H, int V, int max_steps,
                           long long start_token, long long end_token, const float* att1, const float* feat, const float* emb,
                           const float* wz, const float* bz, const float* w_full, const float* b_full,
                           const float* const* wcat, const float* const* beff, const float* Cw, const float* Cb,
                           const float* state0, void* workspace, float* slab, size_t slab_floats, int poll_every,
                           long long* seqs, int* lengths, int* steps_run, int* err_flag, capnet_stream_t stream);

int capnet_att_beam_decode_groups(int cell, int nlayers, int groups, int n, int k, int P, int A, int C, int E, int H, int V,
                                  int max_steps, long long start_token, long long end_token, const float* att1,
                                  const float* feat, const float* emb, const float* wz, const float* bz, const float* w_full,
                                  const float* b_full, const float* const* wcat, const float* const* beff, const float* Cw,
                                  const float* Cb, const float* state0, void* workspace, float* slab, size_t slab_floats,
                                  int poll_every, long long* seqs, int* lengths, int* steps_run, int* err_flag,
                                  capnet_stream_t stream);

size_t capnet_beam_trace_bytes(int n, int k, int max_steps);
int capnet_beam_advance_traced(void* beam, void* trace, const float* logits, long ld, int V, int n, int k, int max_steps,
                               int step, long long end_token, long long* next_words, long long* parent_rows,
                               capnet_stream_t stream);
int capnet_beam_finish_traced(const void* beam, const void* trace, int n, int k, int max_steps, long long end_token,
                              long long* seqs, int* lengths, int* rows, capnet_stream_t stream);

int capnet_att_decode_step_alphas(int cell, int nlayers, int groups, int n, int k, int P, int A, int C, int E, int H, int V,
                                  const float* att1, const float* feat, const long long* tokens, const float* emb,
                                  const float* wz, const float* bz, const float* w_full, const float* b_full,
                                  const float* const* wcat, const float* const* beff, const float* state_in,
                                  const long long* parent_rows, float* state_out, float* h_top, void* workspace, float* slab,
                                  size_t slab_floats, int* err_flag, capnet_stream_t stream, float* alphas);

size_t capnet_att_beam_decode_alphas_ws_bytes(int nlayers, int groups, int n, int k, int P, int A, int C, int E, int H, int V,
                                              int max_steps);
int capnet_att_beam_decode_alphas(int cell, int nlayers, int groups, int n, int k, int P, int A, int C, int E, int H, int V,
                                  int max_steps, long long start_token, long long end_token, const float* att1,
                                  const float* feat, const float* emb, const float* wz, const float* bz, const float* w_full,
                                  const float* b_full, const float* const* wcat, const float* const* beff, const float* Cw,
                                  const float* Cb, const float* state0, void* workspace, float* slab, size_t slab_floats,
                                  int poll_every, long long* seqs, int* lengths, int* steps_run, int* err_flag,
                                  capnet_stream_t stream, float* alphas);

int capnet_beam_nbest(const void* beam, int n, int k, int max_steps, float length_penalty, long long* seqs, int* lengths,
                      float* scores, int* counts, capnet_stream_t stream);
int capnet_beam_nbest_traced(const void* beam, const void* trace, int n, int k, int max_steps, float length_penalty,
                             long long* seqs, int* lengths, float* scores, int* counts, int* rows, capnet_stream_t stream);

size_t capnet_beam_decode_ws_beam_offset(int nlayers, int n, int k, int H, int V, int max_steps, int fused_topk, int groups);
size_t capnet_att_beam_decode_alphas_ws_trace_offset(int nlayers, int groups, int n, int k, int P, int A, int C, int E, int H,
                                                     int V, int max_steps);
size_t capnet_att_beam_decode_alphas_ws_hist_offset(int nlayers, int groups, int n, int k, int P, int A, int C, int E, int H,
                                                    int V, int max_steps);

int capnet_alpha_gather(const float* hist, const int* rows, int captions, int nk, int max_steps, int P, float* alphas,
                        capnet_stream_t stream);

size_t capnet_lstm_wfrag_floats(int H);
int capnet_lstm_pack_wfrag(const float* w_cat, float* w_frag, int H, int cell,
                           capnet_stream_t stream);
int capnet_lstm_step_fused(const float* h_prev, const float* w_frag, float* gates, long ldg,
                           const float* c_prev, float* c_out, float* h_out, int b, int H, int cell,
                           capnet_stream_t stream);
int capnet_lstm_step_fused_stamped(const float* h_prev, const float* w_frag, float* gates, long ldg,
                                   const float* c_prev, float* c_out, float* h_out, int b, int H,
                                   unsigned long long* stamps, capnet_stream_t stream);
int capnet_lstm_step_fused_supported(int b, int H);

int capnet_lstm_persist_supported(int b, int H);
int capnet_lstm_persist_set_mode(int mode);
size_t capnet_lstm_persist_w_floats(void);
size_t capnet_lstm_persist_ctl_ints(void);
int capnet_lstm_persist_pack(const float* w_cat, float* w_img, int cell, capnet_stream_t stream);
int capnet_lstm_persist_run(const float* w_img, float* gates, float* cell_states, float* hiddens,
                            const int* batch_sizes, int t0, int t1, int H, int cell, int segment,
                            int* ctl, int* err_flag, unsigned long long* stamps,
                            capnet_stream_t stream);

int capnet_xent_fwd(const float* logits, long ld, int N, int V, const long long* targets,
                    float* lse, float* row_loss, float* loss, int* err_flag,
                    capnet_stream_t stream);
int capnet_xent_bwd(const float* logits, long ld, int N, int V, const long long* targets,
                    const float* lse, const float* grad_out, float* dlogits, long ldd,
                    capnet_stream_t stream);
int capnet_att_loss_fwd(const float* nll, const float* alphas, int B, int steps, int P, float alpha_c,
                        float* colsum, float* out, capnet_stream_t stream);
int capnet_att_loss_bwd(const float* gout, const float* colsum, int B, int steps, int P, float alpha_c,
                        float* dalphas, capnet_stream_t stream);
int capnet_policy_xent_fwd(const float* logits, long ld, int N, int V, const long long* targets,
                           const float* advantages, int B, const int* batch_sizes, int steps, float* lse,
                           float* row_logp, float* caption_logp, float* loss, int* err_flag, capnet_stream_t stream);
int capnet_policy_xent_bwd(const float* logits, long ld, int N, int V, const long long* targets, const float* lse,
                           const float* advantages, int B, const int* batch_sizes, int steps, const float* grad_out,
                           float* dlogits, long ldd, capnet_stream_t stream);
int capnet_bleu_rows(const long long* ids, long ld, int rows, int steps, long long start_token, long long end_token,
                     int per_image, const int* refs, const int* ref_len, int images, int R, int Lr, const double* weights,
                     int smooth, float* reward, int* stats, capnet_stream_t stream);
int capnet_cider_rows(const long long* ids, long ld, int rows, int steps, long long start_token, long long end_token,
                      int per_image, const int* refs, const int* ref_len, const double* ref_norm, int images, int R, int Lr,
                      const int* const* keys, const double* const* idf, const int* counts, double log_n, double sigma,
                      float* reward, double* parts, int* stats, capnet_stream_t stream);

int capnet_resize_u8(const unsigned char* src, int Hs, int Ws, unsigned char* tmp, unsigned char* dst,
                     int Ho, int Wo, const int* bounds_h, const int* coef_h, int kmax_h,
                     const int* bounds_v, const int* coef_v, int kmax_v, capnet_stream_t stream);
int capnet_crop_flip_normalize(const unsigned char* src, int B, int Hs, int Ws, const int* params,
                               float* dst, int Hc, int Wc, const float* mean, const float* stdv,
                               capnet_stream_t stream);

int capnet_topk_correct(const float* logits, long ld, int N, int V, const long long* targets, int k,
                        int* count, int* err_flag, capnet_stream_t stream);

int capnet_clamp_adam(int n, float* const* params, float* const* grads, float* const* exp_avg,
                      float* const* exp_avg_sq, const long* numel, const int* step, float lr,
                      float beta1, float beta2, float eps, float clip, int write_grad,
                      const int* skip_flag, capnet_stream_t stream);

int capnet_packed_targets(const long long* captions, int T, int steps, const int* batch_sizes,
                          long long* out, capnet_stream_t stream);

int capnet_pack_tensors(int n, float* const* tensors, const long* numel, float* flat,
                        int direction, float scale, capnet_stream_t stream);

size_t capnet_fused_block_weight_words(int C, int MID, int role);
int capnet_fused_block_pack(const float* w, unsigned* img, int C, int MID, int role, capnet_stream_t stream);
size_t capnet_fused_block_stats_floats(long M, int MID);
int capnet_fused_block_stats(const float* y2, const float* s2, const float* t2, const unsigned* w3img, long M, int MID,
                             int in_exp, const float* gamma, const float* beta, float* running_mean, float* running_var,
                             float momentum, float eps, float* scale, float* shift, float* work, int* err_flag,
                             capnet_stream_t stream);
int capnet_fused_block_tiles(long M, int MID);
int capnet_fused_block_forward(const float* y2, const float* s2, const float* t2, const unsigned* w3img, const float* s3,
                               const float* t3, const float* res, const float* sd, const float* td, float* out,
                               const unsigned* w1img, float* y1, float* part_sum, float* part_sq, long M, int MID, int e3,
                               int e1, int* err_flag, capnet_stream_t stream);

typedef struct capnet_comm capnet_comm_t;
int capnet_comm_unique_id(void* id128);
int capnet_comm_create(const void* id128, int rank, int world, capnet_comm_t** out);
int capnet_comm_destroy(capnet_comm_t* comm);
int capnet_allreduce_grads(capnet_comm_t* comm, float* flat, long count, capnet_stream_t stream);

int capnet_err_word_exchange(int* err_flag, float* slot, int direction, capnet_stream_t stream);

int capnet_count_skipped(const int* err_flag, int* counter, capnet_stream_t stream);

int capnet_clamp(float* x, long n, float lo, float hi, capnet_stream_t stream);

#ifdef __cplusplus
}
#endif
#endif
```

Measured before the change: 9103.

## Add persistent BPTT kernel for the LSTM backward recurrence

Replaces the per-timestep loop of pointwise-backward plus recurrent GEMM launches in the decoder LSTM backward with a single persistent kernel. Blocks synchronise across timesteps through global control flags, which removes per-step launch overhead and lets the recurrent weights stay resident. It also makes the forward persistent kernel's shard count configurable, defaulting to a count derived from the batch size rather than a fixed eight. The trade-offs are cross-block spin synchronisation with a timeout/err_flag fallback, extra scratch for the packed weight image, and a different numeric path for the recurrent gradient.

```diff
diff --git a/image-caption-emotion-indonesia_amd/_lib.py b/image-caption-emotion-indonesia_amd/_lib.py
--- a/image-caption-emotion-indonesia_amd/_lib.py
+++ b/image-caption-emotion-indonesia_amd/_lib.py
@@ -106,6 +106,8 @@
                                         C.POINTER(_vp), C.POINTER(_vp), _vp, C.POINTER(_vp), _vp, _vp]),
     "capnet_seq_backward_stacked": (_i, [_ip, _i, _ip, _vp, C.POINTER(_vp), C.POINTER(_vp), C.POINTER(_vp), _vp, C.POINTER(_vp),
                                          C.POINTER(_vp), C.c_float, C.c_ulonglong, _i, _vp]),
+    "capnet_seq_backward_stacked_checked": (_i, [_ip, _i, _ip, _vp, C.POINTER(_vp), C.POINTER(_vp), C.POINTER(_vp), _vp,
+                                                 C.POINTER(_vp), C.POINTER(_vp), C.c_float, C.c_ulonglong, _i, _vp, _vp]),
     "capnet_att_saved_floats": (_sz, [_ip]),
     "capnet_att_saved_ints": (_sz, [_ip]),
     "capnet_att_fwd_scratch_floats": (_sz, [_ip]),
@@ -252,6 +254,12 @@
                                C.POINTER(_vp), C.POINTER(_l), _ip, C.c_float, C.c_float,
                                C.c_float, C.c_float, C.c_float, _i, _vp, _vp]),
     "capnet_lstm_persist_set_mode": (_i, [_i]),
+    "capnet_lstm_persist_set_shards": (_i, [_i]),
+    "capnet_lstm_persist_bwd_supported": (_i, [_i, _i]),
+    "capnet_lstm_persist_bwd_w_floats": (_sz, []),
+    "capnet_lstm_persist_bwd_ctl_ints": (_sz, []),
+    "capnet_lstm_persist_bwd_pack": (_i, [_vp, _vp, _vp]),
+    "capnet_lstm_persist_bwd_run": (_i, [_vp, _vp, _vp, _vp, _vp, _vp, _vp, _ip, _i, _i, _i, _i, _vp, _vp, _vp]),
     "capnet_att_set_chain_mode": (_i, [_i]),
     "capnet_lstm_pointwise_bwd": (_i, [_vp, _vp, _vp, _vp, _vp, _vp, _i, _i, _i, _vp]),
     "capnet_conv1x1_fwd_areg": (_i, [_vp, _vp, _i, _vp, _vp, _vp, _i, _vp, _vp, _l, _i, _i, _i, _vp]),
diff --git a/image-caption-emotion-indonesia_amd/csrc/capi.cpp b/image-caption-emotion-indonesia_amd/csrc/capi.cpp
--- a/image-caption-emotion-indonesia_amd/csrc/capi.cpp
+++ b/image-caption-emotion-indonesia_amd/csrc/capi.cpp
@@ -1193,6 +1193,26 @@
                           f ? 2 : 3, f ? 3 : 2, f ? 0 : 1, segment, ctl, err_flag, S(stream), stamps);
 }
 
+int capnet_lstm_persist_set_shards(int shards) { return lstm_persist_set_shards(shards); }
+int capnet_lstm_persist_bwd_supported(int b, int H) { return lstm_persist_bwd_supported(b, H) ? 1 : 0; }
+size_t capnet_lstm_persist_bwd_w_floats(void) { return lstm_persist_bwd_w_floats(); }
+size_t capnet_lstm_persist_bwd_ctl_ints(void) { return lstm_persist_bwd_ctl_ints(); }
+int capnet_lstm_persist_bwd_pack(const float* w_cat, float* w_img, capnet_stream_t stream) {
+  return lstm_persist_bwd_pack(w_cat, w_img, S(stream));
+}
+int capnet_lstm_persist_bwd_run(const float* w_img, const float* gates, const float* cell_states, const float* d_hiddens,
+                                float* d_pre, float* dh0, float* dc0, const int* batch_sizes, int steps, int lead, int H,
+                                int cell, int* ctl, int* err_flag, capnet_stream_t stream) {
+  CAPNET_REQUIRE(cell == kCellFactored || cell == kCellLSTM, "lstm_persist_bwd_run: unknown cell %d", cell);
+  CAPNET_REQUIRE(batch_sizes && steps > 0 && steps <= kMaxSteps, "lstm_persist_bwd_run: bad steps");
+  int off[kMaxSteps + 1];
+  off[0] = 0;
+  for (int t = 0; t < steps; ++t) off[t + 1] = off[t] + batch_sizes[t];
+  const bool f = cell == kCellFactored;
+  return lstm_persist_bwd_run(w_img, gates, cell_states, d_hiddens, d_pre, dh0, dc0, off, batch_sizes, steps, lead, H, 0, 1,
+                              f ? 2 : 3, f ? 3 : 2, f ? 0 : 1, ctl, err_flag, S(stream));
+}
+
 size_t capnet_seq_saved_floats(const int* dims) { return seq_saved_floats(to_dims(dims)); }
 size_t capnet_seq_saved_ints(const int* dims) { return seq_saved_ints(to_dims(dims)); }
 size_t capnet_seq_saved_cell_offset(const int* dims) { return seq_saved_cell_offset(to_dims(dims)); }
@@ -1226,6 +1246,17 @@
   for (int l = 0; l < nlayers; ++l) to_grads(grads + 9 * l, g[l]);
   return seq_backward_stacked(to_dims(dims), nlayers, batch_sizes, d_hiddens, hiddens, saved, saved_i, scratch, dh_work, g,
                               dropout_p, seed, training, S(stream));
+}
+int capnet_seq_backward_stacked_checked(const int* dims, int nlayers, const int* batch_sizes, const float* d_hiddens,
+                                        const float* const* hiddens, const float* const* saved, const int* const* saved_i,
+                                        float* scratch, float* const* dh_work, float* const* grads, float dropout_p,
+                                        unsigned long long seed, int training, int* err_flag, capnet_stream_t stream) {
+  CAPNET_REQUIRE(dims && grads && err_flag && nlayers >= 1 && nlayers <= 8,
+                 "seq_backward_stacked_checked: null dims / grads / err_flag or layers %d", nlayers);
+  SeqGrads g[8];
+  for (int l = 0; l < nlayers; ++l) to_grads(grads + 9 * l, g[l]);
+  return seq_backward_stacked(to_dims(dims), nlayers, batch_sizes, d_hiddens, hiddens, saved, saved_i, scratch, dh_work, g,
+                              dropout_p, seed, training, S(stream), err_flag);
 }
 
 int capnet_seq_forward(const int* dims, const int* batch_sizes, const unsigned char* tf_mask,
diff --git a/image-caption-emotion-indonesia_amd/csrc/decoder_seq.cpp b/image-caption-emotion-indonesia_amd/csrc/decoder_seq.cpp
--- a/image-caption-emotion-indonesia_amd/csrc/decoder_seq.cpp
+++ b/image-caption-emotion-indonesia_amd/csrc/decoder_seq.cpp
@@ -93,6 +93,8 @@
   S.skws = take(kSplitKFloats);
   S.A1c = take(fac && lead ? N * 4 * F : 0);
   S.A2c = take(fac && lead ? N * 4 * F : 0);
+  S.Wpb = take(H == 512 ? lstm_persist_bwd_w_floats() : 0);
+  S.pctl = take(H == 512 ? lstm_persist_bwd_ctl_ints() : 0);
   S.total = take.o;
   return S;
 }
@@ -337,7 +339,7 @@
 static int seq_backward_layer(const SeqDims& d, const int* batch_sizes, const float* dH, const float* hiddens,
                               const float* saved, const int* saved_i, float* scratch, const SeqGrads& g,
                               float dropout_p, unsigned long long seed, int training, int layer, float* dH_below,
-                              hipStream_t s, int lead = 0, float* dh0 = nullptr, float* dc0 = nullptr) {
+                              hipStream_t s, int lead = 0, float* dh0 = nullptr, float* dc0 = nullptr, int* err_flag = nullptr) {
   RC(check_dims(d, batch_sizes));
   CAPNET_REQUIRE(dH && hiddens && saved && saved_i && scratch, "seq_backward: null argument");
   CAPNET_REQUIRE(g.dWcat && g.dbUW && g.dVcat && (layer > 0 ? dH_below != nullptr : g.dEmb != nullptr), "seq_backward: null gradient buffer");
@@ -352,11 +354,18 @@
   float *dPre = scratch + S.dPre, *Hprev = scratch + S.Hprev, *dh_rec = scratch + S.dh_rec, *dc = scratch + S.dc;
   float *dX = scratch + S.dX, *dA2 = scratch + S.dA2, *dA1 = scratch + S.dA1, *skws = scratch + S.skws;
   const float* sv = saved;
-  CAPNET_HIP_CHECK(hipMemsetAsync(dh_rec, 0, (size_t)d.B * H * sizeof(float), s));
-  CAPNET_HIP_CHECK(hipMemsetAsync(dc, 0, (size_t)d.B * H * sizeof(float), s));
+  const bool persist = err_flag && d.steps <= kMaxSteps && lstm_persist_bwd_supported(batch_sizes[0], H);
+  if (persist) {
+    RC(lstm_persist_bwd_pack(sv + L.Wcat, scratch + S.Wpb, s));
+    RC(lstm_persist_bwd_run(scratch + S.Wpb, sv + L.G, sv + L.Cst, dH, dPre, dh0, dc0, off.data(), batch_sizes, d.steps, lead, H,
+                            go.gi, go.gf, go.go, go.gg, go.tanh_out, reinterpret_cast<int*>(scratch + S.pctl), err_flag, s));
+  } else {
+    CAPNET_HIP_CHECK(hipMemsetAsync(dh_rec, 0, (size_t)d.B * H * sizeof(float), s));
+    CAPNET_HIP_CHECK(hipMemsetAsync(dc, 0, (size_t)d.B * H * sizeof(float), s));
+  }
 
   int slabs = 0;
-  for (int t = d.steps - 1; t >= lead; --t) {
+  for (int t = d.steps - 1; t >= lead && !persist; --t) {
     const int b = batch_sizes[t], r0 = off[t];
     const int b_next = (t + 1 < d.steps) ? batch_sizes[t + 1] : 0;
     RC(lstm_pointwise_bwd(sv + L.G + (size_t)r0 * 4 * H, 4 * H, sv + L.Cst + (size_t)r0 * H,
@@ -373,7 +382,7 @@
                         dh_rec, H, nullptr, 0, skws, kSplitKFloats, s));
     }
   }
-  if (lead) {
+  if (lead && !persist) {
     if (slabs) RC(reduce_slabs(skws, slabs, batch_sizes[0], H, dh_rec, H, nullptr, 0, s));
     RC(copy_d2d(dh0, dh_rec, (size_t)batch_sizes[0] * H, s));
     RC(copy_d2d(dc0, dc, (size_t)batch_sizes[0] * H, s));
@@ -406,15 +415,15 @@
 int seqd::seq_backward_upper(const SeqDims& d, const int* batch_sizes, const float* dH, const float* hiddens,
                              const float* saved, const int* saved_i, float* scratch, const SeqGrads& g, float dropout_p,
                              unsigned long long seed, int training, int layer, float* dH_below, float* dh0, float* dc0,
-                             hipStream_t s) {
+                             hipStream_t s, int* err_flag) {
   return seq_backward_layer(d, batch_sizes, dH, hiddens, saved, saved_i, scratch, g, dropout_p, seed, training, layer,
-                            dH_below, s, 1, dh0, dc0);
+                            dH_below, s, 1, dh0, dc0, err_flag);
 }
 
 int seq_backward_stacked(const SeqDims& d0, int nlayers, const int* batch_sizes, const float* dH_top,
                          const float* const* hiddens, const float* const* saved, const int* const* saved_i, float* scratch,
                          float* const* dH_work, const SeqGrads* g, float dropout_p, unsigned long long seed, int training,
-                         hipStream_t s) {
+                         hipStream_t s, int* err_flag) {
   CAPNET_REQUIRE(nlayers >= 1 && nlayers <= 8 && hiddens && saved && saved_i && g && (nlayers == 1 || dH_work),
                  "seq_backward_stacked: bad argument");
   const float* dH = dH_top;
@@ -422,7 +431,7 @@
     const SeqDims d = l == 0 ? d0 : upper_dims(d0);
     float* below = l > 0 ? dH_work[l - 1] : nullptr;
     RC(seq_backward_layer(d, batch_sizes, dH, hiddens[l], saved[l], saved_i[l], scratch, g[l], dropout_p, seed, training, l,
-                          below, s));
+                          below, s, 0, nullptr, nullptr, err_flag));
     dH = below;
   }
   return kOk;
diff --git a/image-caption-emotion-indonesia_amd/csrc/kernels.h b/image-caption-emotion-indonesia_amd/csrc/kernels.h
--- a/image-caption-emotion-indonesia_amd/csrc/kernels.h
+++ b/image-caption-emotion-indonesia_amd/csrc/kernels.h
@@ -344,6 +344,15 @@
                      const int* batch_sizes, int t0, int t1, int H, int gi, int gf, int go, int gg,
                      int tanh_out, int seg, int* ctl, int* err_flag, hipStream_t stream,
                      unsigned long long* stamps);
+int lstm_persist_set_shards(int shards);
+int lstm_persist_shards(int b);
+bool lstm_persist_bwd_supported(int b, int H);
+size_t lstm_persist_bwd_w_floats();
+size_t lstm_persist_bwd_ctl_ints();
+int lstm_persist_bwd_pack(const float* Wcat, float* Wp, hipStream_t stream);
+int lstm_persist_bwd_run(const float* Wp, const float* G, const float* Cst, const float* dH, float* dPre, float* dh0, float* dc0,
+                         const int* off, const int* batch_sizes, int steps, int lead, int H, int gi, int gf, int go, int gg,
+                         int tanh_out, int* ctl, int* err_flag, hipStream_t stream);
 
 int att_step_fwd(const float* att1, const float* feat, const float* att2, float* gate_io, long ldz,
                  const float* wf, const float* bf, int rows, int P, int A, int C,
@@ -456,7 +465,7 @@
 int seq_backward_stacked(const SeqDims& d0, int nlayers, const int* batch_sizes, const float* dH_top,
                          const float* const* hiddens, const float* const* saved, const int* const* saved_i, float* scratch,
                          float* const* dH_work, const SeqGrads* g, float dropout_p, unsigned long long seed, int training,
-                         hipStream_t s);
+                         hipStream_t s, int* err_flag = nullptr);
 
 struct AttDims {
   int B, T, steps, N, E, F, H, V, A, P, C;
diff --git a/image-caption-emotion-indonesia_amd/csrc/lstm_persist.hip b/image-caption-emotion-indonesia_amd/csrc/lstm_persist.hip
--- a/image-caption-emotion-indonesia_amd/csrc/lstm_persist.hip
+++ b/image-caption-emotion-indonesia_amd/csrc/lstm_persist.hip
@@ -3,6 +3,7 @@
 #include "common.h"
 #include "kernels.h"
 #include "mfma_core.h"
+#include "persist_core.h"
 #include "split_f16.h"
 
 namespace capnet {
@@ -17,7 +18,6 @@
 constexpr int kCtlXcc = kPGrid * 4;
 constexpr int kCtlAbort = kCtlXcc + kPGrid;
 constexpr int kCtlInts = 2048;
-constexpr int kSpinBound = 1 << 21;
 
 struct PersistArgs {
   const float* Wp;
@@ -27,24 +27,14 @@
   int* ctl;
   int* err_flag;
   unsigned long long* stamps;
-  int t0, t1, cfg, seg;
+  int t0, t1, cfg, seg, shards;
   int off[kMaxSteps + 1];
   short b[kMaxSteps];
 };
 
-__device__ __forceinline__ int ld_sc1_i32(const int* p) {
-  return __hip_atomic_load(p, __ATOMIC_RELAXED, __HIP_MEMORY_SCOPE_AGENT);
-}
-__device__ __forceinline__ void st_sc1_i32(int* p, int v) {
-  __hip_atomic_store(p, v, __ATOMIC_RELAXED, __HIP_MEMORY_SCOPE_AGENT);
-}
-__device__ __forceinline__ void st_sc1_f32(float* p, float v) {
-  __hip_atomic_store(p, v, __ATOMIC_RELAXED, __HIP_MEMORY_SCOPE_AGENT);
-}
 template <int OFF> __device__ __forceinline__ void ld16_sc1(f32x4& dst, const float* p) {
   asm volatile("global_load_dwordx4 %0, %1, off offset:%2 sc1" : "=v"(dst) : "v"(p), "n"(OFF) : "memory");
 }
-__device__ __forceinline__ void wait_vm0() { asm volatile("s_waitcnt vmcnt(0)" ::: "memory"); }
 
 constexpr int kWExp = 10;
 __device__ __forceinline__ void p_split8(const f32x4& x0, const f32x4& x1, h8& hi, h8& lo) {
@@ -112,7 +102,8 @@
   __shared__ __attribute__((aligned(16))) float red[2][4][kPMaxRows][68];
   __shared__ int s_local, s_abort;
   const int tid = threadIdx.x, lane = tid & 63, wave = tid >> 6;
-  const int shard = blockIdx.x & 7, slot = blockIdx.x >> 3;
+  const int S = a.shards;
+  const int shard = blockIdx.x % S, slot = blockIdx.x / S;
   const int lm = lane & 15, kq = lane >> 4;
   int* ctl = a.ctl;
   const int gi = a.cfg & 3, gf = (a.cfg >> 2) & 3, go = (a.cfg >> 4) & 3, gg = (a.cfg >> 6) & 3;
@@ -159,7 +150,7 @@
   if (tid == 0 && blockIdx.x == 0 && reinterpret_cast<const unsigned*>(a.Wp)[4l * kPH * kPH] != 0u) atomicOr(a.err_flag, 32);
 
   const int em = tid >> 4, eu = tid & 15;
-  const int grow = 8 * em + shard;
+  const int grow = S * em + shard;
   float c_reg = 0.f;
   if (a.t0 > 0 && grow < a.b[a.t0 - 1])
     c_reg = a.Cst[(long)(a.off[a.t0 - 1] + grow) * H + u0 + eu];
@@ -194,7 +185,7 @@
     unsigned long long ts[6] = {0, 0, 0, 0, 0, 0};
     if (DIAG) ts[0] = __builtin_amdgcn_s_memtime();
     const int bt = b_of(t);
-    const int rows_t = (bt - shard + 7) >> 3;
+    const int rows_t = (bt - shard + S - 1) / S;
     const int ro = off_of(t);
     const bool evalid = em < rows_t;
     const long erow = ro + (evalid ? grow : 0);
@@ -217,7 +208,7 @@
       }
       if (DIAG) ts[1] = __builtin_amdgcn_s_memtime();
       const int rp = off_of(t - 1);
-      const float* hrow = a.hiddens + (long)(rp + 8 * lm + shard) * H + 128 * wave + 4 * kq;
+      const float* hrow = a.hiddens + (long)(rp + S * lm + shard) * H + 128 * wave + 4 * kq;
       if (lm < rows_t) {
         ld16_sc1<0>(hv[0], hrow);
         ld16_sc1<64>(hv[1], hrow);
@@ -334,14 +325,29 @@
 size_t lstm_persist_ctl_ints() { return kCtlInts; }
 
 static int& persist_mode() {
-  static int mode = [] { const char* off = getenv("CAPNET_NO_PERSISTENT_LSTM"); return (off && off[0] == '1') ? 1 : 0; }();
+  static int mode = [] {
+    const char* off = getenv("CAPNET_NO_PERSISTENT_LSTM");
+    const char* boff = getenv("CAPNET_NO_PERSISTENT_BPTT");
+    return ((off && off[0] == '1') ? 1 : 0) | ((boff && boff[0] == '1') ? 8 : 0);
+  }();
   return mode;
 }
 int lstm_persist_set_mode(int mode) {
   const int old = persist_mode();
-  if (mode >= 0) persist_mode() = mode & 7;
+  if (mode >= 0) persist_mode() = mode & 31;
   return old;
 }
+
+static int& persist_shards() {
+  static int shards = [] { const char* v = getenv("CAPNET_PERSISTENT_SHARDS"); return (v && v[0] == '8') ? kPersistGridEight : kPersistGridBatch; }();
+  return shards;
+}
+int lstm_persist_set_shards(int shards) {
+  const int old = persist_shards();
+  if (shards >= 0) persist_shards() = shards == kPersistGridEight ? kPersistGridEight : kPersistGridBatch;
+  return old;
+}
+int lstm_persist_shards(int b) { return persist_shards() == kPersistGridEight ? kPShards : (b + kPMaxRows - 1) / kPMaxRows; }
 
 static int persist_device_ok() {
   static int cached = -1;
@@ -362,7 +368,7 @@
 }
 
 bool lstm_persist_supported(int b, int H) {
-  return H == kPH && b >= 1 && b <= 8 * kPMaxRows && !(persist_mode() & 1) && persist_device_ok();
+  return H == kPH && b >= 1 && b <= kPShards * kPMaxRows && !(persist_mode() & (1 | 16)) && persist_device_ok();
 }
 
 int lstm_persist_pack(const float* Wcat, float* Wp, int gi, int gf, int go, int gg, hipStream_t stream) {
@@ -389,6 +395,7 @@
   a.Wp = Wp; a.G = G; a.Cst = Cst; a.hiddens = hiddens; a.ctl = ctl; a.err_flag = err_flag;
   a.stamps = stamps;
   a.t0 = t0; a.t1 = t1; a.seg = seg;
+  a.shards = lstm_persist_shards(b0);
   a.cfg = gi | (gf << 2) | (go << 4) | (gg << 6) | ((tanh_out ? 1 : 0) << 8) | ((persist_mode() & 2) ? 512 : 0) |
           ((persist_mode() & 4) ? 1024 : 0);
   for (int t = 0; t <= t1; ++t) a.off[t] = off[t];
@@ -398,8 +405,8 @@
     prev = batch_sizes[t];
   }
   for (int t = 0; t < t1; ++t) a.b[t] = (short)batch_sizes[t];
-  if (stamps) hipLaunchKernelGGL((lstm_persist_kernel<true>), dim3(kPGrid), dim3(256), 0, stream, a);
-  else hipLaunchKernelGGL((lstm_persist_kernel<false>), dim3(kPGrid), dim3(256), 0, stream, a);
+  if (stamps) hipLaunchKernelGGL((lstm_persist_kernel<true>), dim3(a.shards * kPSlots), dim3(256), 0, stream, a);
+  else hipLaunchKernelGGL((lstm_persist_kernel<false>), dim3(a.shards * kPSlots), dim3(256), 0, stream, a);
   CAPNET_LAUNCH_CHECK();
   return kOk;
 }
diff --git a/image-caption-emotion-indonesia_amd/csrc/lstm_persist_bwd.hip b/image-caption-emotion-indonesia_amd/csrc/lstm_persist_bwd.hip
--- /dev/null
+++ b/image-caption-emotion-indonesia_amd/csrc/lstm_persist_bwd.hip
@@ -0,0 +1,284 @@
+#include "common.h"
+#include "kernels.h"
+#include "persist_core.h"
+#include "step_core.h"
+
+namespace capnet {
+
+constexpr int kBH = 512;
+constexpr int kBK = 4 * kBH;
+constexpr int kBSlots = 32;
+constexpr int kBUnits = 16;
+constexpr int kBRows = 16;
+constexpr int kBMaxShards = 8;
+constexpr int kBCtlFlags = 0;
+constexpr int kBCtlXcc = kBMaxShards * kBSlots * 4;
+constexpr int kBCtlAbort = kBCtlXcc + kBMaxShards * kBSlots;
+constexpr int kBCtlInts = 2048;
+
+struct PersistBwdArgs {
+  const float* Wp;
+  const float* G;
+  const float* Cst;
+  const float* dH;
+  float* dPre;
+  float* dh0;
+  float* dc0;
+  int* ctl;
+  int* err_flag;
+  unsigned dpre_bytes;
+  int steps, lead, cfg, shards;
+  int off[kMaxSteps + 1];
+  short b[kMaxSteps];
+};
+
+typedef unsigned u32x4 __attribute__((ext_vector_type(4)));
+
+__global__ __launch_bounds__(256) void lstm_persist_bwd_kernel(const PersistBwdArgs a) {
+  constexpr int H = kBH;
+  __shared__ float red[2][4][kBRows][17];
+  __shared__ int s_off[kMaxSteps + 1], s_b[kMaxSteps + 1];
+  __shared__ int s_local, s_abort;
+  const int tid = threadIdx.x, lane = tid & 63, wave = tid >> 6;
+  const int S = a.shards;
+  const int shard = blockIdx.x % S, slot = blockIdx.x / S;
+  const int lm = lane & 15, kq = lane >> 4;
+  int* ctl = a.ctl;
+  const int gi = a.cfg & 3, gf = (a.cfg >> 2) & 3, go = (a.cfg >> 4) & 3, gg = (a.cfg >> 6) & 3;
+  const int tanh_out = (a.cfg >> 8) & 1;
+  const int u0 = slot * kBUnits;
+  const int steps = a.steps, lead = a.lead;
+
+  f32x4 wq[32];
+  {
+    const f32x4* wp = reinterpret_cast<const f32x4*>(a.Wp) + ((long)(slot * 4 + wave) * 32) * 64 + lane;
+#pragma unroll
+    for (int q = 0; q < 32; ++q) wq[q] = wp[(long)q * 64];
+  }
+  for (int i = tid; i <= steps; i += 256) {
+    s_off[i] = a.off[i];
+    s_b[i] = i < steps ? a.b[i] : 0;
+  }
+  if (tid == 0) {
+    s_abort = 0;
+    unsigned x;
+    asm volatile("s_getreg_b32 %0, hwreg(HW_REG_XCC_ID)" : "=s"(x));
+    st_sc1_i32(&ctl[kBCtlXcc + shard * kBSlots + slot], 16 | (int)(x & 15));
+  }
+  if (wave == 0) {
+    int spins = 0, ok = 0, same = 0;
+    while (true) {
+      const int v = ld_sc1_i32(&ctl[kBCtlXcc + shard * kBSlots + (lane & 31)]);
+      const int mine = __shfl(v, slot, 64);
+      ok = __all((v >> 4) == 1);
+      same = __all(v == mine);
+      if (ok) break;
+      if (++spins > kSpinBound || ((spins & 255) == 0 && ld_sc1_i32(&ctl[kBCtlAbort]) != 0)) break;
+      __builtin_amdgcn_s_sleep(4);
+    }
+    if (a.cfg & 1024) ok = 0;
+    if (lane == 0) {
+      s_local = ok && same && !(a.cfg & 512);
+      if (!ok) {
+        s_abort = 1;
+        st_sc1_i32(&ctl[kBCtlAbort], 1);
+        atomicOr(a.err_flag, 4);
+      }
+    }
+  }
+  __syncthreads();
+  if (s_abort) return;
+  const bool local = s_local != 0;
+  if (tid == 0 && slot == 0) ctl[kBCtlAbort + 1 + shard] = local ? 1 : 2;
+
+  const int em = tid >> 4, eu = tid & 15;
+  const int grow = S * em + shard;
+  const int unit = u0 + eu;
+  float dc_reg = 0.f, dh_reg = 0.f;
+  const int* my_flags = ctl + kBCtlFlags + (shard * kBSlots + 8 * wave) * 4 + (lane & 31);
+  int* out_flag = ctl + kBCtlFlags + (shard * kBSlots + slot) * 4 + wave;
+  const __amdgpu_buffer_rsrc_t dpre_rsrc = __builtin_amdgcn_make_buffer_rsrc(a.dPre, 0, a.dpre_bytes, 0x00020000);
+  const int R0 = s_off[lead];
+
+  struct StepIn { float i, f, o, g, ct, cp, dh; };
+  auto load_step = [&](int t, StepIn& in) {
+    if (t < lead || grow >= s_b[t]) return;
+    const long row = s_off[t] + grow;
+    const float* p = a.G + row * (4 * H) + unit;
+    in.i = p[gi * H], in.f = p[gf * H], in.o = p[go * H], in.g = p[gg * H];
+    in.ct = a.Cst[row * H + unit];
+    in.cp = t > 0 ? a.Cst[(long)(s_off[t - 1] + grow) * H + unit] : 0.f;
+    in.dh = a.dH[(row - R0) * H + unit];
+  };
+  StepIn cur = {0.f, 0.f, 0.f, 0.f, 0.f, 0.f, 0.f};
+  load_step(steps - 1, cur);
+
+  for (int t = steps - 1; t >= lead; --t) {
+    const int bt = s_b[t], bnext = s_b[t + 1], ro = s_off[t];
+    const int rows_t = bt > shard ? (bt - shard + S - 1) / S : 0;
+    if (rows_t == 0) {
+      load_step(t - 1, cur);
+      continue;
+    }
+    if (grow < bt) {
+      const long row = ro + grow;
+      const float i = cur.i, f = cur.f, o = cur.o, g = cur.g, ct = cur.ct, cp = cur.cp;
+      float dh = cur.dh;
+      float dc = 0.f;
+      if (grow < bnext) {
+        dh += dh_reg;
+        dc = dc_reg;
+      }
+      float d_o;
+      if (tanh_out) {
+        const float tc = tanhf(ct);
+        d_o = dh * tc;
+        dc += dh * o * (1.f - tc * tc);
+      } else {
+        d_o = dh * ct;
+        dc += dh * o;
+      }
+      const float di = dc * g, dg = dc * i, df = dc * cp;
+      float* q = a.dPre + row * (4 * H) + unit;
+      const float qi = di * i * (1.f - i), qf = df * f * (1.f - f), qo = d_o * o * (1.f - o), qg = dg * (1.f - g * g);
+      if (local) {
+        q[gi * H] = qi;
+        q[gf * H] = qf;
+        q[go * H] = qo;
+        q[gg * H] = qg;
+      } else {
+        st_sc1_f32(q + gi * H, qi);
+        st_sc1_f32(q + gf * H, qf);
+        st_sc1_f32(q + go * H, qo);
+        st_sc1_f32(q + gg * H, qg);
+      }
+      dc_reg = dc * f;
+    }
+    if (t == 0) break;
+    wait_vm0();
+    const int tick = steps - t;
+    if (lane == 0) {
+      if (local) *out_flag = tick;
+      else st_sc1_i32(out_flag, tick);
+    }
+    asm volatile("" ::: "memory");
+    load_step(t - 1, cur);
+    {
+      int spins = 0;
+      while (true) {
+        const int v = ld_sc1_i32(my_flags);
+        if (__all(v - tick >= 0)) break;
+        if (++spins > kSpinBound || ((spins & 255) == 0 && ld_sc1_i32(&ctl[kBCtlAbort]) != 0)) {
+          if (lane == 0) {
+            st_sc1_i32(&ctl[kBCtlAbort], 1);
+            atomicOr(a.err_flag, 4);
+          }
+          break;
+        }
+      }
+    }
+    asm volatile("" ::: "memory");
+    const int prow = ro + (lm < rows_t ? S * lm + shard : shard);
+    const unsigned vo = ((unsigned)prow * kBK + 128 * wave + 4 * kq) * 4u;
+    f32x4 acc[4];
+#pragma unroll
+    for (int e = 0; e < 4; ++e) acc[e] = f32x4{0.f, 0.f, 0.f, 0.f};
+    f32x4 hv[32];
+#pragma unroll
+    for (int r = 0; r < 32; ++r) {
+      const u32x4 raw = __builtin_amdgcn_raw_buffer_load_b128(dpre_rsrc, vo + ((r >> 3) * H + 16 * (r & 7)) * 4u, 0, 16 );
+      hv[r] = __builtin_bit_cast(f32x4, raw);
+    }
+    __builtin_amdgcn_sched_barrier(0);
+#pragma unroll
+    for (int r = 0; r < 32; ++r)
+#pragma unroll
+      for (int e = 0; e < 4; ++e) acc[e] = __builtin_amdgcn_mfma_f32_16x16x4f32(hv[r][e], wq[r][e], acc[e], 0, 0, 0);
+    const f32x4 d = (acc[0] + acc[1]) + (acc[2] + acc[3]);
+#pragma unroll
+    for (int r = 0; r < 4; ++r) red[t & 1][wave][4 * kq + r][lm] = d[r];
+    __syncthreads();
+    dh_reg = sum_partials<4, kBRows>(red[t & 1], em, eu, 0.f);
+  }
+  if (lead > 0 && grow < s_b[0]) {
+    const bool alive = grow < s_b[lead];
+    a.dh0[(long)grow * H + unit] = alive ? dh_reg : 0.f;
+    a.dc0[(long)grow * H + unit] = alive ? dc_reg : 0.f;
+  }
+}
+
+__global__ __launch_bounds__(256) void lstm_persist_bwd_pack_kernel(const float* __restrict__ Wcat, float* __restrict__ Wp) {
+  const long total = (long)kBK * kBH;
+  for (long i = (long)blockIdx.x * blockDim.x + threadIdx.x; i < total; i += (long)gridDim.x * blockDim.x) {
+    const int e = (int)(i & 3), lane = (int)((i >> 2) & 63);
+    long r = i >> 8;
+    const int q = (int)(r & 7); r >>= 3;
+    const int g = (int)(r & 3); r >>= 2;
+    const int w = (int)(r & 3);
+    const int slot = (int)(r >> 2);
+    const int n = lane & 15, kq = lane >> 4;
+    const int k = kBH * g + 128 * w + 16 * q + 4 * kq + e;
+    Wp[i] = Wcat[(long)k * kBH + kBUnits * slot + n];
+  }
+}
+
+size_t lstm_persist_bwd_w_floats() { return (size_t)kBK * kBH; }
+size_t lstm_persist_bwd_ctl_ints() { return kBCtlInts; }
+
+static int persist_bwd_device_ok() {
+  static int cached = -1;
+  if (cached >= 0) return cached;
+  int dev = 0, cus = 0, per_cu = 0;
+  if (hipGetDevice(&dev) != hipSuccess ||
+      hipDeviceGetAttribute(&cus, hipDeviceAttributeMultiprocessorCount, dev) != hipSuccess ||
+      hipOccupancyMaxActiveBlocksPerMultiprocessor(&per_cu, (const void*)lstm_persist_bwd_kernel, 256, 0) != hipSuccess) {
+    (void)hipGetLastError();
+    return cached = 0;
+  }
+  return cached = (cus >= kBMaxShards * kBSlots && per_cu >= 1) ? 1 : 0;
+}
+
+bool lstm_persist_bwd_supported(int b, int H) {
+  return H == kBH && b >= 1 && b <= kBMaxShards * kBRows && !(lstm_persist_set_mode(-1) & (kPersistOff | kPersistBwdOff)) &&
+         persist_bwd_device_ok();
+}
+
+int lstm_persist_bwd_pack(const float* Wcat, float* Wp, hipStream_t stream) {
+  CAPNET_REQUIRE(Wcat && Wp && aligned16(Wp), "lstm_persist_bwd_pack: bad argument");
+  hipLaunchKernelGGL(lstm_persist_bwd_pack_kernel, dim3(1024), dim3(256), 0, stream, Wcat, Wp);
+  CAPNET_LAUNCH_CHECK();
+  return kOk;
+}
+
+int lstm_persist_bwd_run(const float* Wp, const float* G, const float* Cst, const float* dH, float* dPre, float* dh0, float* dc0,
+                         const int* off, const int* batch_sizes, int steps, int lead, int H, int gi, int gf, int go, int gg,
+                         int tanh_out, int* ctl, int* err_flag, hipStream_t stream) {
+  CAPNET_REQUIRE(Wp && G && Cst && dH && dPre && off && batch_sizes && ctl && err_flag, "lstm_persist_bwd_run: null argument");
+  CAPNET_REQUIRE(steps >= 1 && steps <= kMaxSteps && (lead == 0 || lead == 1) && lead < steps,
+                 "lstm_persist_bwd_run: steps %d, lead %d", steps, lead);
+  CAPNET_REQUIRE(lead == 0 || (dh0 && dc0), "lstm_persist_bwd_run: the leading state step needs dh0 and dc0");
+  CAPNET_REQUIRE(lstm_persist_bwd_supported(batch_sizes[0], H), "lstm_persist_bwd_run: unsupported b=%d H=%d", batch_sizes[0], H);
+  CAPNET_REQUIRE(aligned16(Wp) && aligned16(dPre), "lstm_persist_bwd_run: alignment");
+  PersistBwdArgs a;
+  a.Wp = Wp; a.G = G; a.Cst = Cst; a.dH = dH; a.dPre = dPre; a.dh0 = dh0; a.dc0 = dc0; a.ctl = ctl; a.err_flag = err_flag;
+  a.steps = steps; a.lead = lead;
+  const int mode = lstm_persist_set_mode(-1);
+  a.cfg = gi | (gf << 2) | (go << 4) | (gg << 6) | ((tanh_out ? 1 : 0) << 8) | ((mode & kPersistSafe) ? 512 : 0) |
+          ((mode & kPersistInjectTimeout) ? 1024 : 0);
+  a.shards = lstm_persist_shards(batch_sizes[0]);
+  int prev = 1 << 30;
+  for (int t = 0; t < steps; ++t) {
+    CAPNET_REQUIRE(batch_sizes[t] >= 1 && batch_sizes[t] <= prev, "lstm_persist_bwd_run: batch sizes must not grow");
+    CAPNET_REQUIRE(off[t + 1] - off[t] == batch_sizes[t], "lstm_persist_bwd_run: row offsets");
+    prev = batch_sizes[t];
+    a.b[t] = (short)batch_sizes[t];
+  }
+  for (int t = 0; t <= steps; ++t) a.off[t] = off[t];
+  a.dpre_bytes = (unsigned)off[steps] * (unsigned)(kBK * sizeof(float));
+  CAPNET_HIP_CHECK(hipMemsetAsync(ctl, 0, kBCtlInts * sizeof(int), stream));
+  hipLaunchKernelGGL(lstm_persist_bwd_kernel, dim3(a.shards * kBSlots), dim3(256), 0, stream, a);
+  CAPNET_LAUNCH_CHECK();
+  return kOk;
+}
+
+}
diff --git a/image-caption-emotion-indonesia_amd/csrc/persist_core.h b/image-caption-emotion-indonesia_amd/csrc/persist_core.h
--- /dev/null
+++ b/image-caption-emotion-indonesia_amd/csrc/persist_core.h
@@ -0,0 +1,22 @@
+#pragma once
+#include "common.h"
+
+namespace capnet {
+
+constexpr int kSpinBound = 1 << 21;
+
+__device__ __forceinline__ int ld_sc1_i32(const int* p) {
+  return __hip_atomic_load(p, __ATOMIC_RELAXED, __HIP_MEMORY_SCOPE_AGENT);
+}
+__device__ __forceinline__ void st_sc1_i32(int* p, int v) {
+  __hip_atomic_store(p, v, __ATOMIC_RELAXED, __HIP_MEMORY_SCOPE_AGENT);
+}
+__device__ __forceinline__ void st_sc1_f32(float* p, float v) {
+  __hip_atomic_store(p, v, __ATOMIC_RELAXED, __HIP_MEMORY_SCOPE_AGENT);
+}
+__device__ __forceinline__ void wait_vm0() { asm volatile("s_waitcnt vmcnt(0)" ::: "memory"); }
+
+constexpr int kPersistGridBatch = 0, kPersistGridEight = 8;
+constexpr int kPersistOff = 1, kPersistSafe = 2, kPersistInjectTimeout = 4, kPersistBwdOff = 8, kPersistFwdOff = 16;
+
+}
diff --git a/image-caption-emotion-indonesia_amd/csrc/seq_layers.h b/image-caption-emotion-indonesia_amd/csrc/seq_layers.h
--- a/image-caption-emotion-indonesia_amd/csrc/seq_layers.h
+++ b/image-caption-emotion-indonesia_amd/csrc/seq_layers.h
@@ -95,12 +95,12 @@
 };
 int feed_back(const Feedback& f, const float* h_prev, int b, int r0, float* X, long ldx, const SkWs& k, hipStream_t s);
 
-struct BwdLayout { size_t dPre, Hprev, dh_rec, dc, dX, dA2, dA1, skws, A1c, A2c, total; };
+struct BwdLayout { size_t dPre, Hprev, dh_rec, dc, dX, dA2, dA1, skws, A1c, A2c, Wpb, pctl, total; };
 BwdLayout make_bwd_layout(const SeqDims& d, int lead);
 
 int seq_backward_upper(const SeqDims& d, const int* batch_sizes, const float* dH, const float* hiddens, const float* saved,
                        const int* saved_i, float* scratch, const SeqGrads& g, float dropout_p, unsigned long long seed,
-                       int training, int layer, float* dH_below, float* dh0, float* dc0, hipStream_t s);
+                       int training, int layer, float* dH_below, float* dh0, float* dc0, hipStream_t s, int* err_flag = nullptr);
 
 }
 }
diff --git a/image-caption-emotion-indonesia_amd/ops.py b/image-caption-emotion-indonesia_amd/ops.py
--- a/image-caption-emotion-indonesia_amd/ops.py
+++ b/image-caption-emotion-indonesia_amd/ops.py
@@ -1825,11 +1825,12 @@
             grads += g + [dEmb if l == 0 else None, dFeat if l == 0 else None]
             per_layer.append(g)
         dh_work = [new(N, H) for _ in range(nl - 1)]
-        check(L.capnet_seq_backward_stacked(cd[0], nl, int_array(cfg["batch_sizes"]), ptr(_c(d_hiddens)), ptr_array(hid),
-                                            ptr_array(saved), ptr_array(saved_i), ptr(scratch),
-                                            ptr_array(dh_work) if dh_work else None, ptr_array(grads),
-                                            float(cfg["dropout"]), int(cfg["seed"]), _seq_training(cfg), current_stream()),
-              "capnet_seq_backward_stacked")
+        check(L.capnet_seq_backward_stacked_checked(cd[0], nl, int_array(cfg["batch_sizes"]), ptr(_c(d_hiddens)),
+                                                    ptr_array(hid), ptr_array(saved), ptr_array(saved_i), ptr(scratch),
+                                                    ptr_array(dh_work) if dh_work else None, ptr_array(grads),
+                                                    float(cfg["dropout"]), int(cfg["seed"]), _seq_training(cfg),
+                                                    ptr(err_flag(dev)), current_stream()),
+              "capnet_seq_backward_stacked_checked")
         wg = []
         for g in per_layer:
             wg += _gate_grads(cell, F, H, *g)
diff --git a/include/capnet.h b/include/capnet.h
--- a/include/capnet.h
+++ b/include/capnet.h
@@ -210,6 +210,10 @@
                                 const float* const* hiddens, const float* const* saved, const int* const* saved_i,
                                 float* scratch, float* const* dh_work, float* const* grads, float dropout_p,
                                 unsigned long long seed, int training, capnet_stream_t stream);
+int capnet_seq_backward_stacked_checked(const int* dims, int nlayers, const int* batch_sizes, const float* d_hiddens,
+                                        const float* const* hiddens, const float* const* saved, const int* const* saved_i,
+                                        float* scratch, float* const* dh_work, float* const* grads, float dropout_p,
+                                        unsigned long long seed, int training, int* err_flag, capnet_stream_t stream);
 
 int capnet_att_set_chain_mode(int mode);
 size_t capnet_att_saved_floats(const int* dims);
@@ -518,6 +522,7 @@
 
 int capnet_lstm_persist_supported(int b, int H);
 int capnet_lstm_persist_set_mode(int mode);
+int capnet_lstm_persist_set_shards(int shards);
 size_t capnet_lstm_persist_w_floats(void);
 size_t capnet_lstm_persist_ctl_ints(void);
 int capnet_lstm_persist_pack(const float* w_cat, float* w_img, int cell, capnet_stream_t stream);
@@ -525,6 +530,14 @@
                             const int* batch_sizes, int t0, int t1, int H, int cell, int segment,
                             int* ctl, int* err_flag, unsigned long long* stamps,
                             capnet_stream_t stream);
+
+int capnet_lstm_persist_bwd_supported(int b, int H);
+size_t capnet_lstm_persist_bwd_w_floats(void);
+size_t capnet_lstm_persist_bwd_ctl_ints(void);
+int capnet_lstm_persist_bwd_pack(const float* w_cat, float* w_img, capnet_stream_t stream);
+int capnet_lstm_persist_bwd_run(const float* w_img, const float* gates, const float* cell_states, const float* d_hiddens,
+                                float* d_pre, float* dh0, float* dc0, const int* batch_sizes, int steps, int lead, int H,
+                                int cell, int* ctl, int* err_flag, capnet_stream_t stream);
 
 int capnet_xent_fwd(const float* logits, long ld, int N, int V, const long long* targets,
                     float* lse, float* row_loss, float* loss, int* err_flag,
```

Result: no change. 9100 (-0.0%).
